# ShahzaibAhmad05/NextSearch-api

Hardware: AMD Instinct MI355X
Metric: queries/sec at k=10 over 1M-doc index; achieved HBM GB/s vs peak (higher is better)
Workload: dtype f32

## Files before the change

### include/nextsearch_hip.h

```cpp
#ifndef NEXTSEARCH_HIP_H
#define NEXTSEARCH_HIP_H

#include <stdint.h>

#ifdef __cplusplus
extern "C" {
#endif

#define NS_OK            0
#define NS_E_INVAL      -1
#define NS_E_NODEVICE   -2
#define NS_E_HIP        -3
#define NS_E_NOMEM      -4
#define NS_E_STATE      -5

#define NS_MAX_K        100u

#define NS_FLAG_OR      0u
#define NS_FLAG_AND     1u
#define NS_INFO_IMPACTS 0x100u
#define NS_INFO_PACKED  0x200u
#define NS_INFO_SHARED  0x800u
#define NS_INFO_PRUNED  0x400u

typedef struct ns_ctx   ns_ctx;
typedef struct ns_seg   ns_seg;
typedef struct ns_batch ns_batch;

typedef struct ns_term_ref {
    uint32_t seg_id;
    uint32_t count;
    uint64_t byte_off;
    float    idf;
    float    qweight;
} ns_term_ref;

typedef struct ns_query_desc {
    uint32_t term_begin;
    uint32_t term_count;
} ns_query_desc;

typedef struct ns_hit {
    float    score;
    uint32_t seg_id;
    uint32_t doc_id;
} ns_hit;

typedef struct ns_batch_info {
    uint64_t postings;
    uint64_t algo_bytes;
    uint32_t n_queries;
    uint32_t n_items;
    uint32_t n_term_refs;
    uint32_t tile_docs;
    uint32_t k;
    uint32_t flags;
    float    last_score_kernel_ms;
    float    last_total_ms;
    uint32_t timed_runs;
    uint32_t shared_lists;
    double   sum_score_kernel_ms;
    double   sum_total_ms;
    uint64_t shared_postings;
} ns_batch_info;

int  ns_ctx_create(int device, ns_ctx** out);
void ns_ctx_destroy(ns_ctx* ctx);
int  ns_ctx_set_stream(ns_ctx* ctx, void* hip_stream);
const char* ns_last_error(ns_ctx* ctx);
const char* ns_device_name(ns_ctx* ctx);

int ns_segment_upload(ns_ctx* ctx, uint32_t seg_id, uint32_t n_docs, float avgdl,
                      const uint32_t* doc_len, const void* postings, uint64_t nbytes, ns_seg** out);
int ns_segment_release(ns_ctx* ctx, ns_seg* seg);
int ns_segment_upload_begin(ns_ctx* ctx, uint32_t seg_id, uint32_t n_docs, float avgdl, const uint32_t* doc_len,
                            uint64_t total_nbytes, ns_seg** out);
int ns_segment_upload_append(ns_ctx* ctx, ns_seg* seg, const void* bytes, uint64_t nbytes);
int ns_segment_upload_end(ns_ctx* ctx, ns_seg* seg);

int ns_segment_build_impacts(ns_ctx* ctx, ns_seg* seg, const uint64_t* byte_off, const uint32_t* counts,
                             const float* idfs, uint32_t n_lists);
int ns_ctx_set_overlap(ns_ctx* ctx, int on);
int ns_ctx_set_host_threads(ns_ctx* ctx, uint32_t n);
int ns_segment_build_packed(ns_ctx* ctx, ns_seg* seg);
int ns_ctx_use_packed(ns_ctx* ctx, int mode);
int ns_ctx_use_impacts(ns_ctx* ctx, int on);
int ns_segment_build_skips(ns_ctx* ctx, ns_seg* seg, const uint64_t* byte_off, const uint32_t* counts, uint32_t n_lists);
int ns_segment_filter(ns_ctx* ctx, ns_seg* src, uint32_t new_seg_id, const uint32_t* keep_bits, const uint64_t* byte_off,
                      const uint32_t* counts, uint32_t n_lists, uint64_t* new_byte_off_out, uint32_t* new_counts_out,
                      void* postings_out, uint64_t* kept_postings_out, float* device_ms_out, ns_seg** out);
int ns_ctx_use_skips(ns_ctx* ctx, int on);
int ns_segment_build_blockmax(ns_ctx* ctx, ns_seg* seg, const uint64_t* byte_off, const uint32_t* counts,
                              const float* idfs, uint32_t n_lists);
int ns_ctx_use_pruning(ns_ctx* ctx, int on);
int ns_ctx_use_merge(ns_ctx* ctx, int on);
int ns_ctx_share_scores(ns_ctx* ctx, int mode);

int ns_ctx_share_rows(ns_ctx* ctx, int mode);
int ns_batch_row_stats(ns_batch* b, uint32_t out[4]);

int ns_search_batch(ns_ctx* ctx, const ns_query_desc* queries, const ns_term_ref* terms,
                    uint32_t n_queries, uint32_t k, ns_hit* hits_out, uint32_t* nhits_out,
                    uint64_t* found_out, uint32_t flags);

int  ns_batch_prepare(ns_ctx* ctx, const ns_query_desc* queries, const ns_term_ref* terms,
                      uint32_t n_queries, uint32_t k, uint32_t flags, ns_batch** out);
int  ns_batch_bind_outputs(ns_batch* b, void* d_hits, void* d_nhits, void* d_found);
#define NS_RUN_TIMED 1
#define NS_RUN_FETCH 2
int  ns_batch_run(ns_batch* b, int run_flags);
void* ns_batch_stream(ns_batch* b);
int  ns_batch_gap_ms(ns_batch* prev, ns_batch* next, float* ms);
int  ns_batch_sync(ns_batch* b);
int  ns_batch_fetch(ns_batch* b, ns_hit* hits_out, uint32_t* nhits_out, uint64_t* found_out);
int  ns_batch_get_info(ns_batch* b, ns_batch_info* info);
void ns_batch_destroy(ns_batch* b);

typedef struct ns_sem ns_sem;
int ns_sem_upload(ns_ctx* ctx, const float* vecs, uint32_t n_rows, uint32_t dim, ns_sem** out);
int ns_sem_release(ns_ctx* ctx, ns_sem* sem);
int ns_sem_topk(ns_ctx* ctx, ns_sem* sem, const float* qvecs, uint32_t n_q, uint32_t topk, float min_sim,
                const uint32_t* ban_off, const uint32_t* ban_rows, uint32_t* rows_out, float* sims_out,
                uint32_t* counts_out, float* device_ms_out);

typedef struct ns_ac ns_ac;
int ns_ac_upload(ns_ctx* ctx, const uint8_t* pool, const uint64_t* offsets, const uint32_t* scores, uint32_t n_terms, ns_ac** out);
int ns_ac_suggest(ns_ctx* ctx, ns_ac* ac, const uint8_t* prefix_bytes, const uint32_t* prefix_offsets, uint32_t n_q, uint32_t L,
                  uint32_t* idx_out, uint32_t* count_out, float* device_ms_out);
int ns_ac_release(ns_ctx* ctx, ns_ac* ac);

#define NS_FUZZY_MAX_LEN   64u
#define NS_FUZZY_MAX_EDITS 2u
int ns_ac_build_fuzzy(ns_ctx* ctx, ns_ac* ac, float* device_ms_out);
int ns_ac_fuzzy(ns_ctx* ctx, ns_ac* ac, const uint8_t* term_bytes, const uint32_t* term_offsets, uint32_t n_q,
                const uint8_t* max_edits, uint32_t prefix_len, uint32_t L, uint32_t* idx_out, uint8_t* dist_out,
                uint32_t* count_out, float* device_ms_out);

int ns_ac_fuzzy_prefix(ns_ctx* ctx, ns_ac* ac, const uint8_t* prefix_bytes, const uint32_t* prefix_offsets, uint32_t n_q,
                       const uint8_t* max_edits, uint32_t prefix_len, uint32_t L, uint32_t* idx_out, uint8_t* dist_out,
                       uint32_t* count_out, float* device_ms_out);

int ns_merge_rank_rows(ns_ctx* ctx, const void* d_hits, const void* d_nhits, const void* d_found, uint32_t n_ranks,
                       uint32_t n_queries, uint32_t k, const uint32_t* d_seg_map, uint32_t seg_map_stride,
                       void* d_out_hits, void* d_out_nhits, void* d_out_found);

int ns_invert_forward(ns_ctx* ctx, const uint32_t* doc_term_counts, uint32_t n_docs, const uint32_t* pairs,
                      uint64_t n_pairs, uint32_t n_terms, uint32_t* df_out, void* postings_out, uint64_t* kept_out,
                      float* device_ms_out);
int ns_segment_upload_inverted(ns_ctx* ctx, ns_seg* seg, const uint32_t* doc_term_counts, const uint32_t* pairs,
                               uint64_t n_pairs, uint32_t n_terms, uint32_t* df_out, void* postings_out,
                               uint64_t* kept_out, float* device_ms_out);

#define NS_E_ARG NS_E_INVAL
typedef struct ns_forward ns_forward;
typedef struct ns_forward_info {
    uint32_t struct_size;
    uint32_t kept_docs;
    uint32_t n_terms;
    uint32_t n_docs;
    uint64_t n_pairs;
    uint64_t term_bytes;
    uint64_t n_tokens;
    uint64_t kept_tokens;
    uint64_t device_bytes;
    float    device_ms;
    uint32_t pad;
} ns_forward_info;
int ns_forward_build(ns_ctx* ctx, const uint8_t* text, uint64_t text_bytes, const uint64_t* offsets, uint32_t n_docs,
                     ns_forward** out);
int ns_forward_get_info(const ns_forward* fwd, ns_forward_info* info);
int ns_forward_fetch(ns_forward* fwd, uint32_t* kept_docs_out, uint32_t* doc_len_out, uint32_t* counts_out,
                     uint32_t* pairs_out, uint8_t* term_bytes_out, uint64_t* term_offsets_out);
void ns_forward_destroy(ns_forward* fwd);

typedef struct ns_forward_src {
    uint32_t n_docs;  const uint32_t* doc_len;  const uint32_t* counts;
    uint64_t n_pairs; const uint32_t* pairs;
    uint32_t n_terms; const uint8_t* term_bytes; const uint64_t* term_offsets;
} ns_forward_src;
int ns_forward_merge(ns_ctx* ctx, const ns_forward_src* src, uint32_t n_src, ns_forward** out);
int ns_forward_invert(ns_forward* fwd, uint32_t* df_out, void* postings_out, uint64_t* kept_out, float* device_ms_out);
uint32_t ns_compact_doc_cut(void);
// ... 73 lines not shown
```

### nextsearch-api_amd/csrc/ns_api.hip

```cpp
#include <hip/hip_runtime.h>

#include <algorithm>
#include <cmath>
#include <cstdarg>
#include <cstdio>
#include <cstdlib>
#include <cstring>
#include <string>
#include <vector>

#include "../../include/nextsearch_hip.h"
#include "ns_internal.h"
#include "ns_plan.hpp"
#include "ns_kernels.hip"
#include "ns_wave_kernel.hip"
#include "ns_driver_kernel.hip"
#include "ns_prune_kernel.hip"
#include "ns_merge_kernel.hip"
#include "ns_tile_kernel.hip"
#include "ns_row_kernel.hip"
#include "ns_invert.hip"
#include "ns_ingest.hip"
#include "ns_compact.hip"
#include "ns_delete.hip"
#include "ns_filter.hip"
#include "ns_facet.hip"
#include "ns_similar.hip"
#include "ns_sorted.hip"
#include "ns_boolean.hip"
#include "ns_boolean_sets.hip"
#include "ns_sem.hip"
#include "ns_suggest.hip"
#include "ns_fuzzy.hip"

using namespace ns;

static_assert(sizeof(ns_hit) == sizeof(Hit), "ns_hit layout");


struct ns_seg {
    ns_ctx* ctx = nullptr;
    uint32_t id = 0;
    uint32_t n_docs = 0;
    uint64_t n_postings = 0;
    uint2* d_postings = nullptr;
    float* d_norm = nullptr;
    float* d_pnorm = nullptr;
    bool norm_safe = false;
    float avgdl = 0.0f;
    bool pending = false;
    uint64_t filled = 0;
    uint32_t* d_len = nullptr;
    void* pin[2] = {nullptr, nullptr};
    hipEvent_t ev[2] = {nullptr, nullptr};
    int stage_k = 0;
    uint32_t* d_packed = nullptr;
    uint2* d_pk_hdr = nullptr;
    float* d_pk_scores = nullptr;
    uint16_t* d_nidx = nullptr;
    float* d_ntab = nullptr;
    uint32_t n_norms = 0;
    uint2* d_impacts = nullptr;
    uint32_t* d_skips = nullptr;
    std::vector<uint32_t*> skip_retired;
    uint64_t skip_cap = 0, skip_used = 0;
    uint32_t skip_entries() const { return (n_docs + kSkipDocs - 1) / kSkipDocs + 2; }
    float* d_blockmax = nullptr;
    std::vector<float*> bmx_retired;
    uint64_t bmx_cap = 0, bmx_used = 0;
    SegLists lists;
};

struct ns_ctx {
    struct Block { void* p; size_t n; };
    std::vector<Block> pool;
    size_t pool_bytes = 0;
    int device = 0;
    hipStream_t own_stream = nullptr;
    hipStream_t stream = nullptr;
    hipStream_t alt_stream = nullptr;
    hipStream_t pull_stream = nullptr;
    bool overlap = false, flip = false;
    hipStream_t row_stream = nullptr;
    std::string err;
    std::string devname;
    std::vector<ns_seg*> segs;
    std::vector<ns_seg*> pending_uploads;
    void* h_up = nullptr;
    size_t h_up_cap = 0;
    hipEvent_t up_done = nullptr;
    bool up_busy = false;
    void* h_down = nullptr;
    size_t h_down_cap = 0;
    struct ns_batch* down_owner = nullptr;
    struct DownSlot { void* p = nullptr; size_t cap = 0; bool busy = false; };
    std::vector<DownSlot> down_slots;
    PlanSettings cfg;
    ShareRegistry share;
    BatchPlan plan;
    std::vector<ns_ac*> acs;
    std::vector<ns_forward*> fwds;
    bool cp_inplace = true;
    std::vector<ns_docterms*> dts;
};

static thread_local std::string g_create_err;
static void ac_free_fwd(ns_ac* ac);
static void forward_orphan_fwd(ns_forward* f);
static void docterms_orphan_fwd(ns_docterms* h);
static void seg_free_device_fwd(ns_seg* s);
static void seg_free_staging_fwd(ns_seg* s);

static int fail(ns_ctx* ctx, int code, const char* fmt, ...) {
    va_list ap;
    va_start(ap, fmt);
    (ctx ? ctx->err : g_create_err) = vformat(fmt, ap);
    va_end(ap);
    return code;
}

#define HIPCHK(ctx, call)                                                                         \
    do {                                                                                          \
        hipError_t e_ = (call);                                                                   \
        if (e_ != hipSuccess)                                                                     \
            return fail((ctx), NS_E_HIP, "%s failed: %s (%s:%d)", #call, hipGetErrorString(e_), __FILE__, __LINE__); \
    } while (0)

template <int CB, int TMAX, bool IMP, int PK>
static void launch_uscore(bool and_mode, uint32_t n_items, hipStream_t st, const DevWItem* items, const DevTerm* terms,
                          const DevSeg* segs, Hit* hits, uint32_t* nhits, uint64_t* found, uint32_t K) {
    dim3 grid((n_items + kUscoreWavesPerBlock - 1) / kUscoreWavesPerBlock), block(64 * kUscoreWavesPerBlock);
    if (and_mode)
        hipLaunchKernelGGL((k_uscore<512, 192, true, CB, TMAX, IMP, PK>), grid, block, 0, st, items, n_items, terms, segs, hits, nhits, found, K);
    else
        hipLaunchKernelGGL((k_uscore<512, 192, false, CB, TMAX, IMP, PK>), grid, block, 0, st, items, n_items, terms, segs, hits, nhits, found, K);
}
template <int CB, int TMAX>
static void launch_uscore(bool and_mode, bool imp, int pk, uint32_t n_items, hipStream_t st, const DevWItem* items,
                          const DevTerm* terms, const DevSeg* segs, Hit* hits, uint32_t* nhits, uint64_t* found, uint32_t K) {
    if (imp && pk) launch_uscore<CB, TMAX, true, 1>(and_mode, n_items, st, items, terms, segs, hits, nhits, found, K);
    else if (imp) launch_uscore<CB, TMAX, true, 0>(and_mode, n_items, st, items, terms, segs, hits, nhits, found, K);
    else if (pk == 2) launch_uscore<CB, TMAX, false, 2>(and_mode, n_items, st, items, terms, segs, hits, nhits, found, K);
    else if (pk == 1) launch_uscore<CB, TMAX, false, 1>(and_mode, n_items, st, items, terms, segs, hits, nhits, found, K);
    else launch_uscore<CB, TMAX, false, 0>(and_mode, n_items, st, items, terms, segs, hits, nhits, found, K);
}

template <int HK, int FB>
static void launch_dscore(bool and_mode, uint32_t n_items, hipStream_t st, const DevWItem* items, const DevTerm* terms,
                          const DevSeg* segs, Hit* hits, uint32_t* nhits, uint64_t* found, uint32_t K) {
    dim3 grid((n_items + 3) / 4), block(256);
    if (and_mode)
        hipLaunchKernelGGL((k_dscore<HK, FB, true>), grid, block, 0, st, items, n_items, terms, segs, hits, nhits, found, K);
    else
        hipLaunchKernelGGL((k_dscore<HK, FB, false>), grid, block, 0, st, items, n_items, terms, segs, hits, nhits, found, K);
}

template <int TD>
static void launch_tscore(bool and_mode, uint32_t n_items, hipStream_t st, const DevWItem* items, const DevTerm* terms,
                          const DevSeg* segs, Hit* hits, uint32_t* nhits, uint64_t* found, uint32_t K) {
    dim3 grid((n_items + 3) / 4), block(256);
    if (and_mode)
        hipLaunchKernelGGL((k_tscore<TD, true>), grid, block, 0, st, items, n_items, terms, segs, hits, nhits, found, K);
    else
        hipLaunchKernelGGL((k_tscore<TD, false>), grid, block, 0, st, items, n_items, terms, segs, hits, nhits, found, K);
}

template <int NT, int SPT, int U>
static void launch_score(bool and_mode, uint32_t n_items, hipStream_t st, const DevItem* items, const DevTerm* terms,
                         const DevSeg* segs, const uint32_t* bounds, Hit* hits, uint32_t* nhits, uint64_t* found,
                         uint32_t K) {
    if (and_mode)
        hipLaunchKernelGGL((k_score<NT, SPT, U, true>), dim3(n_items), dim3(NT), 0, st, items, terms, segs, bounds, hits, nhits, found, K);
    else
        hipLaunchKernelGGL((k_score<NT, SPT, U, false>), dim3(n_items), dim3(NT), 0, st, items, terms, segs, bounds, hits, nhits, found, K);
}

extern "C" int ns_ctx_create(int device, ns_ctx** out) {
    if (!out) return fail(nullptr, NS_E_INVAL, "ns_ctx_create: out is NULL");
    *out = nullptr;
    int ndev = 0;
    hipError_t e = hipGetDeviceCount(&ndev);
    if (e != hipSuccess || ndev <= 0)
        return fail(nullptr, NS_E_NODEVICE, "no HIP device available (%s); this library has no CPU fallback",
                    e == hipSuccess ? "device count 0" : hipGetErrorString(e));
    if (device < 0 || device >= ndev) return fail(nullptr, NS_E_INVAL, "device %d out of range [0,%d)", device, ndev);
    e = hipSetDevice(device);
    if (e != hipSuccess) return fail(nullptr, NS_E_NODEVICE, "hipSetDevice(%d): %s", device, hipGetErrorString(e));
    hipDeviceProp_t prop;
    e = hipGetDeviceProperties(&prop, device);
    if (e != hipSuccess) return fail(nullptr, NS_E_NODEVICE, "hipGetDeviceProperties: %s", hipGetErrorString(e));
    ns_ctx* ctx = new ns_ctx();
    ctx->device = device;
    ctx->devname = std::string(prop.gcnArchName) + " " + prop.name;
    ctx->cfg.n_cus = prop.multiProcessorCount;
    e = hipStreamCreateWithFlags(&ctx->own_stream, hipStreamNonBlocking);
    if (e != hipSuccess) {
        int rc = fail(nullptr, NS_E_HIP, "hipStreamCreate: %s", hipGetErrorString(e));
        delete ctx;
        return rc;
    }
    ctx->stream = ctx->own_stream;
    if (const char* om = std::getenv("NS_ORDER_MODE")) ctx->cfg.order_mode = std::atoi(om);
    if (const char* kp = std::getenv("NS_KEY_PCT")) {
        unsigned a = 100, b = 100, c = 100, d = 100;
        if (std::sscanf(kp, "%u,%u,%u,%u", &a, &b, &c, &d) >= 1) { ctx->cfg.key_pct[0] = a; ctx->cfg.key_pct[1] = b; ctx->cfg.key_pct[2] = c; ctx->cfg.key_pct[3] = d; }
    }
    if (const char* td = std::getenv("NS_TILE_DENS64")) ctx->cfg.tile_dens64 = (uint32_t)std::max(1, std::atoi(td));
    if (const char* um = std::getenv("NS_MERGE")) ctx->cfg.use_merge = std::atoi(um) != 0;
    if (const char* mr = std::getenv("NS_MERGE_RATIO")) ctx->cfg.merge_ratio = (uint32_t)std::max(1, std::atoi(mr));
    if (const char* sm = std::getenv("NS_SHARE")) ctx->cfg.share_mode = std::max(0, std::min(2, std::atoi(sm)));
    if (const char* sr = std::getenv("NS_SHARE_RATIO")) ctx->cfg.share_ratio = (uint32_t)std::max(1, std::atoi(sr));
    if (const char* sp = std::getenv("NS_SHARE_MIN")) ctx->cfg.share_min_postings = (uint64_t)std::max(0ll, std::atoll(sp));
    ctx->cfg.row_mode = 1;
    if (const char* rm = std::getenv("NS_SHARE_ROWS")) ctx->cfg.row_mode = std::max(0, std::min(2, std::atoi(rm)));
    if (const char* ru = std::getenv("NS_ROW_MIN_USERS")) ctx->cfg.row_min_users = (uint32_t)std::max(1, std::atoi(ru));
    if (const char* rc = std::getenv("NS_ROW_CELL")) ctx->cfg.row_cell_postings = (uint32_t)std::max(1, std::atoi(rc));
    {
        const char* rf = std::getenv("NS_ROW_FORK");
        if ((!rf || std::atoi(rf) != 0) && hipStreamCreateWithFlags(&ctx->row_stream, hipStreamNonBlocking) != hipSuccess) { ctx->row_stream = nullptr; (void)hipGetLastError(); }
    }
    if (const char* oc = std::getenv("NS_ORDER_COARSE")) { ctx->cfg.order_coarse = std::max(0, std::min(11, std::atoi(oc))); ctx->cfg.order_coarse_forced = true; }
    if (hipStreamCreateWithFlags(&ctx->alt_stream, hipStreamNonBlocking) != hipSuccess) { ctx->alt_stream = nullptr; (void)hipGetLastError(); }
    {
        int lo_pri = 0, hi_pri = 0;
        (void)hipDeviceGetStreamPriorityRange(&lo_pri, &hi_pri);
        if (hipStreamCreateWithPriority(&ctx->pull_stream, hipStreamNonBlocking, hi_pri) != hipSuccess) { ctx->pull_stream = nullptr; (void)hipGetLastError(); }
    }
    *out = ctx;
    return NS_OK;
}

extern "C" void ns_ctx_destroy(ns_ctx* ctx) {
    if (!ctx) return;
    (void)hipSetDevice(ctx->device);
    (void)hipStreamSynchronize(ctx->stream);
    if (ctx->alt_stream) (void)hipStreamSynchronize(ctx->alt_stream);
    if (ctx->pull_stream) (void)hipStreamSynchronize(ctx->pull_stream);
    if (ctx->row_stream) (void)hipStreamSynchronize(ctx->row_stream);
    for (ns_seg* s : ctx->segs) {
        if (!s) continue;
        seg_free_device_fwd(s);
        delete s;
    }
    for (ns_seg* s : ctx->pending_uploads) {
        seg_free_staging_fwd(s);
        seg_free_device_fwd(s);
        delete s;
    }
    for (ns_ac* ac : ctx->acs) ac_free_fwd(ac);
    for (ns_forward* f : ctx->fwds) forward_orphan_fwd(f);
    for (ns_docterms* h : ctx->dts) docterms_orphan_fwd(h);
    for (auto& blk : ctx->pool) (void)hipFree(blk.p);
    if (ctx->h_up) (void)hipHostFree(ctx->h_up);
    if (ctx->h_down) (void)hipHostFree(ctx->h_down);
    for (auto& ds : ctx->down_slots) if (ds.p) (void)hipHostFree(ds.p);
    if (ctx->up_done) (void)hipEventDestroy(ctx->up_done);
    if (ctx->own_stream) (void)hipStreamDestroy(ctx->own_stream);
    if (ctx->alt_stream) (void)hipStreamDestroy(ctx->alt_stream);
    if (ctx->pull_stream) (void)hipStreamDestroy(ctx->pull_stream);
    if (ctx->row_stream) (void)hipStreamDestroy(ctx->row_stream);
    delete ctx;
}

extern "C" int ns_ctx_set_stream(ns_ctx* ctx, void* hip_stream) {
    if (!ctx) return fail(nullptr, NS_E_INVAL, "ns_ctx_set_stream: ctx is NULL");
    ctx->stream = hip_stream ? (hipStream_t)hip_stream : ctx->own_stream;
    return NS_OK;
}

extern "C" const char* ns_last_error(ns_ctx* ctx) { return ctx ? ctx->err.c_str() : g_create_err.c_str(); }
extern "C" const char* ns_device_name(ns_ctx* ctx) { return ctx ? ctx->devname.c_str() : ""; }

extern "C" int ns_set_tuning(ns_ctx* ctx, uint32_t variant, uint32_t min_items, uint32_t split_postings) {
    if (!ctx) return fail(nullptr, NS_E_INVAL, "ns_set_tuning: ctx is NULL");
    if (variant >= kNumVariants || kVariants[variant].nt == 0) return fail(ctx, NS_E_INVAL, "unknown kernel variant %u", variant);
#ifndef NS_VARIANTS
    if (variant != 0) return fail(ctx, NS_E_INVAL, "kernel variant %u exists only in the variants build (make -C nextsearch-api_amd variants)", variant);
#endif
    ctx->cfg.variant = variant;
    ctx->cfg.min_items = min_items;
    ctx->cfg.split_postings = split_postings;
    return NS_OK;
}

static constexpr size_t kPadPostings = 256;
static constexpr size_t kStageChunk = 32u << 20;

static void seg_free_staging(ns_seg* s) {
    for (int i = 0; i < 2; i++) {
        if (s->pin[i]) (void)hipHostFree(s->pin[i]);
        if (s->ev[i]) (void)hipEventDestroy(s->ev[i]);
        s->pin[i] = nullptr; s->ev[i] = nullptr;
    }
    if (s->d_len) (void)hipFree(s->d_len);
    s->d_len = nullptr;
}
static void seg_free_device(ns_seg* s);
static void seg_free_device_fwd(ns_seg* s) { seg_free_device(s); }
static void seg_free_staging_fwd(ns_seg* s) { seg_free_staging(s); }
static void seg_free_device(ns_seg* s) {
    (void)hipFree(s->d_postings);
    (void)hipFree(s->d_norm);
    (void)hipFree(s->d_pnorm);
    (void)hipFree(s->d_impacts);
    (void)hipFree(s->d_packed);
    (void)hipFree(s->d_pk_hdr);
    (void)hipFree(s->d_pk_scores);
    (void)hipFree(s->d_nidx);
    (void)hipFree(s->d_ntab);
    (void)hipFree(s->d_skips);
    for (uint32_t* p : s->skip_retired) (void)hipFree(p);
    s->skip_retired.clear();
    (void)hipFree(s->d_blockmax);
    for (float* p : s->bmx_retired) (void)hipFree(p);
    s->bmx_retired.clear();
    s->d_blockmax = nullptr; s->bmx_cap = s->bmx_used = 0; s->lists.bmx.clear();
    s->d_skips = nullptr; s->skip_cap = s->skip_used = 0; s->lists.skip.clear();
    s->d_postings = nullptr; s->d_norm = nullptr; s->d_pnorm = nullptr; s->d_impacts = nullptr; s->d_packed = nullptr;
    s->d_pk_hdr = nullptr; s->d_pk_scores = nullptr; s->d_nidx = nullptr; s->d_ntab = nullptr;
}
static hipError_t seg_stage(ns_ctx* ctx, ns_seg* s, void* dst, const void* src, size_t n) {
    size_t off = 0;
    while (off < n) {
        const size_t c = std::min(kStageChunk, n - off);
        const int k = s->stage_k;
        hipError_t r = hipEventSynchronize(s->ev[k]);
        if (r != hipSuccess) return r;
        std::memcpy(s->pin[k], (const char*)src + off, c);
        r = hipMemcpyAsync((char*)dst + off, s->pin[k], c, hipMemcpyHostToDevice, ctx->stream);
        if (r != hipSuccess) return r;
        r = hipEventRecord(s->ev[k], ctx->stream);
        if (r != hipSuccess) return r;
        off += c;
        s->stage_k ^= 1;
    }
    return hipSuccess;
}

extern "C" int ns_segment_upload_begin(ns_ctx* ctx, uint32_t seg_id, uint32_t n_docs, float avgdl, const uint32_t* doc_len,
                                       uint64_t nbytes, ns_seg** out) {
    if (!ctx) return fail(nullptr, NS_E_INVAL, "ns_segment_upload: ctx is NULL");
    if (!out) return fail(ctx, NS_E_INVAL, "ns_segment_upload_begin: out is NULL");
    *out = nullptr;
    if (seg_id >= (1u << 20)) return fail(ctx, NS_E_INVAL, "seg_id %u too large", seg_id);
    if (nbytes % 8 != 0) return fail(ctx, NS_E_INVAL, "posting payload of %llu bytes is not a whole number of {u32,u32} pairs", (unsigned long long)nbytes);
    if (nbytes / 8 >= (1ull << 32)) return fail(ctx, NS_E_INVAL, "segment has %llu postings; this build indexes postings with 32 bits (split the segment)", (unsigned long long)(nbytes / 8));
    if (n_docs && !doc_len) return fail(ctx, NS_E_INVAL, "null doc_len/postings");
    if (seg_id < ctx->segs.size() && ctx->segs[seg_id]) return fail(ctx, NS_E_INVAL, "segment %u already uploaded", seg_id);
    HIPCHK(ctx, hipSetDevice(ctx->device));

    ns_seg* s = new ns_seg();
    s->ctx = ctx;
    s->id = seg_id;
    s->n_docs = n_docs;
    s->n_postings = nbytes / 8;
    s->avgdl = avgdl;
    s->pending = true;
    auto cleanup = [&]() { seg_free_staging(s); seg_free_device(s); delete s; };

    hipError_t e;
    if ((e = hipMalloc((void**)&s->d_postings, nbytes + kPadPostings * 8)) != hipSuccess) { cleanup(); return fail(ctx, NS_E_NOMEM, "hipMalloc postings (%llu B): %s", (unsigned long long)nbytes, hipGetErrorString(e)); }
    if ((e = hipMalloc((void**)&s->d_norm, (size_t)std::max<uint32_t>(n_docs, 1) * 4)) != hipSuccess) { cleanup(); return fail(ctx, NS_E_NOMEM, "hipMalloc norm: %s", hipGetErrorString(e)); }
    if ((e = hipMalloc((void**)&s->d_pnorm, nbytes / 2 + kPadPostings * 4)) != hipSuccess) { cleanup(); return fail(ctx, NS_E_NOMEM, "hipMalloc per-posting norms (%llu B): %s", (unsigned long long)(nbytes / 2), hipGetErrorString(e)); }
    if ((e = hipMalloc((void**)&s->d_len, (size_t)std::max<uint32_t>(n_docs, 1) * 4)) != hipSuccess) { cleanup(); return fail(ctx, NS_E_NOMEM, "hipMalloc doc_len: %s", hipGetErrorString(e)); }
    for (int i = 0; i < 2; i++)
        if (hipHostMalloc(&s->pin[i], kStageChunk, hipHostMallocDefault) != hipSuccess || hipEventCreateWithFlags(&s->ev[i], hipEventDisableTiming) != hipSuccess) {
            cleanup();
            return fail(ctx, NS_E_NOMEM, "pinned staging allocation failed");
        }
    e = hipMemsetAsync((char*)s->d_postings + nbytes, 0xFF, kPadPostings * 8, ctx->stream);
    if (e == hipSuccess) e = hipMemsetAsync((char*)s->d_pnorm + nbytes / 2, 0, kPadPostings * 4, ctx->stream);
    if (e == hipSuccess && n_docs) e = seg_stage(ctx, s, s->d_len, doc_len, (size_t)n_docs * 4);
    if (e == hipSuccess && n_docs) {
        hipLaunchKernelGGL(k_norm, dim3((n_docs + 255) / 256), dim3(256), 0, ctx->stream, s->d_len, s->d_norm, n_docs, avgdl);
        e = hipGetLastError();
    }
    if (e == hipSuccess && n_docs) {
        uint32_t max_len = 0;
        for (uint32_t i = 0; i < n_docs; i++) max_len = std::max(max_len, doc_len[i]);
        std::vector<uint32_t> uniq;
        std::vector<uint16_t> nidx;
        if (max_len < (1u << 24)) {
            std::vector<uint32_t> rank((size_t)max_len + 1, 0u);
            for (uint32_t i = 0; i < n_docs; i++) rank[doc_len[i]] = 1u;
            for (uint32_t v = 0; v <= max_len; v++)
                if (rank[v]) { rank[v] = (uint32_t)uniq.size(); uniq.push_back(v); }
            if (uniq.size() <= 65536) {
                nidx.resize(n_docs);
                for (uint32_t i = 0; i < n_docs; i++) nidx[i] = (uint16_t)rank[doc_len[i]];
            }
        } else {
            uniq.assign(doc_len, doc_len + n_docs);
            std::sort(uniq.begin(), uniq.end());
            uniq.erase(std::unique(uniq.begin(), uniq.end()), uniq.end());
            if (uniq.size() <= 65536) {
                nidx.resize(n_docs);
                for (uint32_t i = 0; i < n_docs; i++) nidx[i] = (uint16_t)(std::lower_bound(uniq.begin(), uniq.end(), doc_len[i]) - uniq.begin());
            }
        }
        if (!nidx.empty()) {
// ... 222 lines not shown
    }
}

extern "C" int ns_ctx_share_scores(ns_ctx* ctx, int mode) {
    if (!ctx) return fail(nullptr, NS_E_INVAL, "ns_ctx_share_scores: ctx is NULL");
    if (mode < 0 || mode > 2) return fail(ctx, NS_E_INVAL, "ns_ctx_share_scores: mode %d outside [0, 2]", mode);
    ctx->cfg.share_mode = mode;
    return NS_OK;
}

extern "C" int ns_ctx_share_rows(ns_ctx* ctx, int mode) {
    if (!ctx) return fail(nullptr, NS_E_INVAL, "ns_ctx_share_rows: ctx is NULL");
    if (mode < 0 || mode > 2) return fail(ctx, NS_E_INVAL, "ns_ctx_share_rows: mode %d outside [0, 2]", mode);
    ctx->cfg.row_mode = mode;
    return NS_OK;
}

extern "C" int ns_segment_build_packed(ns_ctx* ctx, ns_seg* seg) {
    if (!ctx || !seg) return fail(ctx, NS_E_INVAL, "ns_segment_build_packed: null argument");
    if (seg->pending || seg->id >= ctx->segs.size() || ctx->segs[seg->id] != seg) return fail(ctx, NS_E_INVAL, "segment does not belong to this ctx");
    if (seg->d_packed || !seg->n_postings) return NS_OK;
    if (!seg->d_nidx) return fail(ctx, NS_E_INVAL, "ns_segment_build_packed: segment %u has more than 65536 distinct document lengths; its norms do not fit a 16-bit index", seg->id);
    HIPCHK(ctx, hipSetDevice(ctx->device));
    const uint64_t n_blocks = (seg->n_postings + kPkBlock - 1) / kPkBlock;
    hipError_t e = hipMalloc((void**)&seg->d_packed, (n_blocks + 2) * kPkStrideDwords * 4);
    if (e == hipSuccess) e = hipMalloc((void**)&seg->d_pk_hdr, (n_blocks + 2) * sizeof(uint2));
    if (e == hipSuccess) e = hipMemsetAsync(seg->d_packed + n_blocks * kPkStrideDwords, 0, 2 * kPkStrideDwords * 4, ctx->stream);
    if (e == hipSuccess) e = hipMemsetAsync(seg->d_pk_hdr + n_blocks, 0, 2 * sizeof(uint2), ctx->stream);
    if (e == hipSuccess) {
        hipLaunchKernelGGL(k_pack, dim3((uint32_t)n_blocks), dim3(64), 0, ctx->stream, seg->d_postings, seg->d_nidx, seg->d_packed, seg->d_pk_hdr,
                           seg->n_postings, seg->n_docs, (uint32_t)n_blocks);
        e = hipGetLastError();
    }
    if (e == hipSuccess) e = hipStreamSynchronize(ctx->stream);
    if (e == hipSuccess) e = seg_fill_pk_scores(ctx, seg);
    if (e != hipSuccess) {
        (void)hipFree(seg->d_packed); (void)hipFree(seg->d_pk_hdr);
        seg->d_packed = nullptr; seg->d_pk_hdr = nullptr;
        return fail(ctx, e == hipErrorOutOfMemory ? NS_E_NOMEM : NS_E_HIP, "ns_segment_build_packed: %s", hipGetErrorString(e));
    }
    return NS_OK;
}

__global__ void __launch_bounds__(256) k_skip_fill(uint32_t* __restrict__ sk, const uint32_t* __restrict__ starts, const uint32_t* __restrict__ counts,
                                                   uint32_t per_list) {
    const uint32_t l = blockIdx.y;
    const uint32_t endp = starts[l] + counts[l];
    for (uint32_t i = blockIdx.x * 256 + threadIdx.x; i < per_list; i += gridDim.x * 256) sk[(uint64_t)l * per_list + i] = endp;
}
__global__ void __launch_bounds__(256) k_skip_build(const uint2* __restrict__ postings, uint32_t* __restrict__ sk, const uint32_t* __restrict__ starts,
                                                    const uint32_t* __restrict__ counts, uint32_t per_list) {
    const uint32_t l = blockIdx.y;
    const uint32_t first = starts[l], n = counts[l];
    uint32_t* row = sk + (uint64_t)l * per_list;
    const uint32_t cells = per_list - 2;
    for (uint32_t i = blockIdx.x * 256 + threadIdx.x; i < n; i += gridDim.x * 256) {
        const uint32_t d = postings[first + i].x / kSkipDocs;
        uint32_t c0 = 0;
        if (i) {
            const uint32_t dp = postings[first + i - 1].x / kSkipDocs;
            c0 = dp + 1;
        }
        for (uint32_t c = c0; c <= d && c <= cells; c++) row[c] = first + i;
    }
}
__global__ void __launch_bounds__(256) k_skip_check(const uint2* __restrict__ postings, const uint32_t* __restrict__ sk, const uint32_t* __restrict__ starts,
                                                    const uint32_t* __restrict__ counts, uint32_t per_list, uint32_t* __restrict__ bad) {
    const uint32_t l = blockIdx.y;
    const uint32_t first = starts[l], endp = first + counts[l];
    const uint32_t* row = sk + (uint64_t)l * per_list;
    bool b = false;
    for (uint32_t i = blockIdx.x * 256 + threadIdx.x; i + 1 < per_list; i += gridDim.x * 256) {
        const uint32_t a = row[i], z = row[i + 1];
        if (a > z || a < first || z > endp) b = true;
        if (i == 0 && a != first) b = true;
        if (i + 2 == per_list && (z != endp || a != endp)) b = true;
        if (i + 2 < per_list && a < z) {
            if (postings[a].x / kSkipDocs != i || postings[z - 1].x / kSkipDocs != i) b = true;
        }
    }
    if (b) bad[l] = 1u;
}

extern "C" int ns_segment_build_skips(ns_ctx* ctx, ns_seg* seg, const uint64_t* byte_off, const uint32_t* counts, uint32_t n_lists) {
    if (!ctx || !seg) return fail(ctx, NS_E_INVAL, "ns_segment_build_skips: null argument");
    if (seg->pending || seg->id >= ctx->segs.size() || ctx->segs[seg->id] != seg) return fail(ctx, NS_E_INVAL, "segment does not belong to this ctx");
    if (n_lists && (!byte_off || !counts)) return fail(ctx, NS_E_INVAL, "null list arrays");
    if (!n_lists || !seg->n_postings || !seg->n_docs) return NS_OK;
    HIPCHK(ctx, hipSetDevice(ctx->device));
    if (int rc = check_lists(ctx, seg, byte_off, counts, n_lists)) return rc;
    struct L { uint32_t first, count; };
    std::vector<L> lists;
    lists.reserve(n_lists);
    for (uint32_t i = 0; i < n_lists; i++)
        if (counts[i] && !seg->lists.skip_of((uint32_t)(byte_off[i] / 8), counts[i])) lists.push_back({(uint32_t)(byte_off[i] / 8), counts[i]});
    std::sort(lists.begin(), lists.end(), [](const L& a, const L& b) { return a.first < b.first || (a.first == b.first && a.count < b.count); });
    lists.erase(std::unique(lists.begin(), lists.end(), [](const L& a, const L& b) { return a.first == b.first; }), lists.end());
    if (lists.empty()) return NS_OK;
    const uint32_t per_list = seg->skip_entries();
    const size_t n = lists.size();
    const uint64_t need = seg->skip_used + (uint64_t)n * per_list;
    if (need >= (1ull << 32) - 1) return fail(ctx, NS_E_INVAL, "ns_segment_build_skips: %llu table entries do not fit 32 bits", (unsigned long long)need);
    hipError_t e = hipSuccess;
    if (need > seg->skip_cap) {
        uint32_t* bigger = nullptr;
        const uint64_t cap = std::max<uint64_t>(need, seg->skip_cap * 2);
        e = hipMalloc((void**)&bigger, cap * 4);
        if (e != hipSuccess) return fail(ctx, NS_E_NOMEM, "hipMalloc skip tables (%llu B): %s", (unsigned long long)(cap * 4), hipGetErrorString(e));
        if (seg->d_skips) {
            e = hipMemcpyAsync(bigger, seg->d_skips, seg->skip_used * 4, hipMemcpyDeviceToDevice, ctx->stream);
            seg->skip_retired.push_back(seg->d_skips);
        }
        seg->d_skips = bigger;
        seg->skip_cap = cap;
        if (e != hipSuccess) return fail(ctx, NS_E_HIP, "ns_segment_build_skips: %s", hipGetErrorString(e));
    }
    std::vector<uint32_t> h(n * 3, 0u);
    for (size_t i = 0; i < n; i++) { h[i] = lists[i].first; h[n + i] = lists[i].count; }
    uint32_t* d_tmp = nullptr;
    e = hipMalloc((void**)&d_tmp, n * 12);
    if (e == hipSuccess) e = hipMemcpyAsync(d_tmp, h.data(), n * 12, hipMemcpyHostToDevice, ctx->stream);
    uint32_t* base = seg->d_skips + seg->skip_used;
    if (e == hipSuccess) {
        const dim3 g1((per_list + 255) / 256 > 64 ? 64 : (per_list + 255) / 256, (uint32_t)n);
        hipLaunchKernelGGL(k_skip_fill, g1, dim3(256), 0, ctx->stream, base, d_tmp, d_tmp + n, per_list);
        uint32_t cmax = 0;
        for (const auto& l : lists) cmax = std::max(cmax, l.count);
        const dim3 g2(std::min<uint32_t>((cmax + 255) / 256, 1024u), (uint32_t)n);
        hipLaunchKernelGGL(k_skip_build, g2, dim3(256), 0, ctx->stream, seg->d_postings, base, d_tmp, d_tmp + n, per_list);
        hipLaunchKernelGGL(k_skip_check, g1, dim3(256), 0, ctx->stream, seg->d_postings, base, d_tmp, d_tmp + n, per_list, d_tmp + 2 * n);
        e = hipGetLastError();
    }
    std::vector<uint32_t> bad(n, 1u);
    if (e == hipSuccess) e = hipMemcpyAsync(bad.data(), d_tmp + 2 * n, n * 4, hipMemcpyDeviceToHost, ctx->stream);
    if (e == hipSuccess) e = hipStreamSynchronize(ctx->stream);
    (void)hipFree(d_tmp);
    if (e != hipSuccess) return fail(ctx, NS_E_HIP, "ns_segment_build_skips: %s", hipGetErrorString(e));
    for (size_t i = 0; i < n; i++)
        if (!bad[i] && !seg->lists.skip.find(lists[i].first)) seg->lists.skip.put(lists[i].first, {lists[i].count, (uint32_t)(seg->skip_used + i * per_list)});
    seg->skip_used = need;
    return NS_OK;
}

extern "C" int ns_segment_build_blockmax(ns_ctx* ctx, ns_seg* seg, const uint64_t* byte_off, const uint32_t* counts, const float* idfs, uint32_t n_lists) {
    if (!ctx || !seg) return fail(ctx, NS_E_INVAL, "ns_segment_build_blockmax: null argument");
    if (seg->pending || seg->id >= ctx->segs.size() || ctx->segs[seg->id] != seg) return fail(ctx, NS_E_INVAL, "segment does not belong to this ctx");
    if (n_lists && (!byte_off || !counts || !idfs)) return fail(ctx, NS_E_INVAL, "null list arrays");
    if (!n_lists || !seg->n_postings) return NS_OK;
    HIPCHK(ctx, hipSetDevice(ctx->device));
    if (int rc = check_lists(ctx, seg, byte_off, counts, n_lists)) return rc;
    struct L { uint32_t first, count; float idf; uint32_t entry; };
    std::vector<L> lists;
    lists.reserve(n_lists);
    for (uint32_t i = 0; i < n_lists; i++) {
        uint32_t ib; std::memcpy(&ib, &idfs[i], 4);
        if (counts[i] && !seg->lists.bmx_of((uint32_t)(byte_off[i] / 8), counts[i], ib)) lists.push_back({(uint32_t)(byte_off[i] / 8), counts[i], idfs[i], 0u});
    }
    std::sort(lists.begin(), lists.end(), [](const L& a, const L& b) { return a.first < b.first; });
    lists.erase(std::unique(lists.begin(), lists.end(), [](const L& a, const L& b) { return a.first == b.first; }), lists.end());
    if (lists.empty()) return NS_OK;
    uint64_t need = seg->bmx_used;
    uint32_t bmax_blocks = 0;
    for (auto& l : lists) {
        const uint32_t nb = (l.count + kBmxBlock - 1) / kBmxBlock;
        l.entry = (uint32_t)need;
        need += nb;
        bmax_blocks = std::max(bmax_blocks, nb);
    }
    if (need + 64 >= (1ull << 32) - 1) return fail(ctx, NS_E_INVAL, "ns_segment_build_blockmax: %llu entries do not fit 32 bits", (unsigned long long)need);
    hipError_t e = hipSuccess;
    if (need + 64 > seg->bmx_cap) {
        float* bigger = nullptr;
        const uint64_t cap = std::max<uint64_t>(need + 64, seg->bmx_cap * 2);
        e = hipMalloc((void**)&bigger, cap * 4);
        if (e != hipSuccess) return fail(ctx, NS_E_NOMEM, "hipMalloc block maxima (%llu B): %s", (unsigned long long)(cap * 4), hipGetErrorString(e));
        e = hipMemsetAsync(bigger, 0, cap * 4, ctx->stream);
        if (e == hipSuccess && seg->d_blockmax) {
            e = hipMemcpyAsync(bigger, seg->d_blockmax, seg->bmx_used * 4, hipMemcpyDeviceToDevice, ctx->stream);
            seg->bmx_retired.push_back(seg->d_blockmax);
        }
        seg->d_blockmax = bigger;
        seg->bmx_cap = cap;
        if (e != hipSuccess) return fail(ctx, NS_E_HIP, "ns_segment_build_blockmax: %s", hipGetErrorString(e));
    }
    const size_t n = lists.size();
    std::vector<uint32_t> h(n * 4);
    for (size_t i = 0; i < n; i++) {
        h[i] = lists[i].first; h[n + i] = lists[i].count;
        std::memcpy(&h[2 * n + i], &lists[i].idf, 4);
        h[3 * n + i] = lists[i].entry;
    }
    uint32_t* d_tmp = nullptr;
    e = hipMalloc((void**)&d_tmp, n * 16);
    if (e == hipSuccess) e = hipMemcpyAsync(d_tmp, h.data(), n * 16, hipMemcpyHostToDevice, ctx->stream);
    if (e == hipSuccess) {
        for (size_t l0 = 0; l0 < n; l0 += 32768) {
            const uint32_t ny = (uint32_t)std::min<size_t>(32768, n - l0);
            hipLaunchKernelGGL(k_blockmax, dim3(std::min<uint32_t>(std::max<uint32_t>(bmax_blocks, 1u), 256u), ny), dim3(64), 0, ctx->stream,
                               seg->d_postings, seg->d_pnorm, seg->d_blockmax, d_tmp + l0, d_tmp + n + l0, (const float*)(d_tmp + 2 * n + l0), d_tmp + 3 * n + l0);
        }
        e = hipGetLastError();
    }
    if (e == hipSuccess) e = hipStreamSynchronize(ctx->stream);
    (void)hipFree(d_tmp);
    if (e != hipSuccess) return fail(ctx, NS_E_HIP, "ns_segment_build_blockmax: %s", hipGetErrorString(e));
    seg->bmx_used = need;
    for (const auto& l : lists) {
        uint32_t ib; std::memcpy(&ib, &l.idf, 4);
        seg->lists.bmx.put(l.first, {l.count, ib, l.entry});
    }
    return NS_OK;
}

extern "C" int ns_ctx_use_merge(ns_ctx* ctx, int on) {
    if (!ctx) return NS_E_INVAL;
    ctx->cfg.use_merge = on != 0;
    return NS_OK;
}

extern "C" int ns_ctx_use_pruning(ns_ctx* ctx, int on) {
    if (!ctx) return NS_E_INVAL;
    ctx->cfg.use_pruning = on != 0;
    return NS_OK;
// ... 542 lines not shown
    if (!b) return NS_E_INVAL;
    ns_ctx* ctx = b->ctx;
    HIPCHK(ctx, hipSetDevice(ctx->device));
    HIPCHK(ctx, hipStreamSynchronize(b->st));
    return batch_collect_timings(b);
}

extern "C" int ns_batch_fetch(ns_batch* b, ns_hit* hits_out, uint32_t* nhits_out, uint64_t* found_out) {
    if (!b) return NS_E_INVAL;
    ns_ctx* ctx = b->ctx;
    if (!b->ran) return fail(ctx, NS_E_STATE, "ns_batch_fetch before ns_batch_run");
    HIPCHK(ctx, hipSetDevice(ctx->device));
    hipStream_t st = b->st;
    const bool own_outputs = b->o_hits == b->d_hits && b->o_nhits == b->d_nhits && b->o_found == b->d_found;
    if (b->fetch_enqueued && b->done_recorded && own_outputs) {
        HIPCHK(ctx, hipEventSynchronize(b->done));
        int rc = batch_collect_timings(b);
        if (rc != NS_OK) return rc;
        if (b->Q) {
            const char* h = (ctx->down_owner == b) ? (const char*)ctx->h_down : (const char*)ctx->down_slots[(size_t)b->down_slot].p;
            if (hits_out) std::memcpy(hits_out, h, (size_t)b->Q * b->K * sizeof(Hit));
            if (nhits_out) std::memcpy(nhits_out, h + b->off_nhits, (size_t)b->Q * 4);
            if (found_out) std::memcpy(found_out, h + b->off_found, (size_t)b->Q * 8);
        }
        if (b->down_slot >= 0) { ctx->down_slots[(size_t)b->down_slot].busy = false; b->down_slot = -1; }
        b->fetch_enqueued = false;
        return NS_OK;
    }
    if (b->Q && own_outputs && ctx->down_owner == b) {
        int rc = ns_batch_sync(b);
        if (rc != NS_OK) return rc;
        const char* h = (const char*)ctx->h_down;
        if (hits_out) std::memcpy(hits_out, h, (size_t)b->Q * b->K * sizeof(Hit));
        if (nhits_out) std::memcpy(nhits_out, h + b->off_nhits, (size_t)b->Q * 4);
        if (found_out) std::memcpy(found_out, h + b->off_found, (size_t)b->Q * 8);
        return NS_OK;
    }
    if (b->Q && own_outputs && !ctx->down_owner && b->out_span <= kStageMaxBytes) {
        if (ctx->h_down_cap < b->out_span) {
            if (ctx->h_down) (void)hipHostFree(ctx->h_down);
            ctx->h_down = nullptr; ctx->h_down_cap = 0;
            const size_t cap = std::max<size_t>(b->out_span + b->out_span / 2, 1 << 16);
            if (hipHostMalloc(&ctx->h_down, cap, hipHostMallocDefault) == hipSuccess) ctx->h_down_cap = cap;
            else { ctx->h_down = nullptr; (void)hipGetLastError(); }
        }
        if (ctx->h_down_cap >= b->out_span) {
            HIPCHK(ctx, hipMemcpyAsync(ctx->h_down, b->d_hits, b->out_span, hipMemcpyDeviceToHost, st));
            int rc = ns_batch_sync(b);
            if (rc != NS_OK) return rc;
            const char* h = (const char*)ctx->h_down;
            if (hits_out) std::memcpy(hits_out, h, (size_t)b->Q * b->K * sizeof(Hit));
            if (nhits_out) std::memcpy(nhits_out, h + b->off_nhits, (size_t)b->Q * 4);
            if (found_out) std::memcpy(found_out, h + b->off_found, (size_t)b->Q * 8);
            return NS_OK;
        }
    }
    if (b->Q) {
        if (hits_out) HIPCHK(ctx, hipMemcpyAsync(hits_out, b->o_hits, (size_t)b->Q * b->K * sizeof(Hit), hipMemcpyDeviceToHost, st));
        if (nhits_out) HIPCHK(ctx, hipMemcpyAsync(nhits_out, b->o_nhits, (size_t)b->Q * 4, hipMemcpyDeviceToHost, st));
        if (found_out) HIPCHK(ctx, hipMemcpyAsync(found_out, b->o_found, (size_t)b->Q * 8, hipMemcpyDeviceToHost, st));
    }
    return ns_batch_sync(b);
}

extern "C" int ns_batch_get_info(ns_batch* b, ns_batch_info* info) {
    if (!b || !info) return NS_E_INVAL;
    info->postings = b->postings;
    info->algo_bytes = b->postings * 8;
    info->n_queries = b->Q;
    info->n_items = b->n_items + b->n_witems + b->n_ritems + b->n_pitems;
    info->n_term_refs = b->n_terms;
    info->tile_docs = b->tile_docs;
    info->k = b->K;
    info->flags = b->flags | (b->imp ? NS_INFO_IMPACTS : 0u) | (b->pk ? NS_INFO_PACKED : 0u) | (b->pruned ? NS_INFO_PRUNED : 0u) |
                  (b->shared ? NS_INFO_SHARED : 0u);
    info->shared_lists = b->n_share;
    info->shared_postings = b->share_postings;
    info->last_score_kernel_ms = b->last_score_ms;
    info->last_total_ms = b->last_total_ms;
    info->timed_runs = b->timed_runs;
    info->sum_score_kernel_ms = b->sum_score_ms;
    info->sum_total_ms = b->sum_total_ms;
    return NS_OK;
}

extern "C" int ns_batch_row_stats(ns_batch* b, uint32_t out[4]) {
    if (!b || !out) return NS_E_INVAL;
    ns_ctx* ctx = b->ctx;
    const bool rows = b->n_pitems && b->n_ritems && b->variant == 0;
    out[0] = rows ? b->n_pitems : 0u; out[1] = rows ? b->n_ritems : 0u; out[2] = 0u; out[3] = 0u;
    if (rows && b->ran) {
        HIPCHK(ctx, hipSetDevice(ctx->device));
        HIPCHK(ctx, hipMemcpyAsync(out + 2, b->d_row_stats, 8, hipMemcpyDeviceToHost, b->st));
        HIPCHK(ctx, hipStreamSynchronize(b->st));
    }
    return NS_OK;
}

extern "C" int ns_search_batch(ns_ctx* ctx, const ns_query_desc* queries, const ns_term_ref* terms, uint32_t n_queries,
                               uint32_t k, ns_hit* hits_out, uint32_t* nhits_out, uint64_t* found_out, uint32_t flags) {
    ns_batch* b = nullptr;
    int rc = ns_batch_prepare(ctx, queries, terms, n_queries, k, flags, &b);
    if (rc != NS_OK) return rc;
    rc = ns_batch_run(b, 0);
    if (rc == NS_OK) rc = ns_batch_fetch(b, hits_out, nhits_out, found_out);
    ns_batch_destroy(b);
    return rc;
}


static int invert_run(ns_ctx* ctx, const uint32_t* doc_term_counts, uint32_t n_docs, const uint32_t* pairs,
                      uint64_t n_pairs, uint32_t n_terms, uint32_t* df_out, void* postings_out, uint64_t* kept_out,
                      float* device_ms_out, ns_seg* adopt, const uint2* dev_pairs = nullptr) {
    if (!ctx) return fail(nullptr, NS_E_INVAL, "ns_invert_forward: ctx is NULL");
    if ((n_docs && !doc_term_counts) || (n_pairs && !pairs && !dev_pairs) || (n_terms && !df_out) || !kept_out) return fail(ctx, NS_E_INVAL, "ns_invert_forward: null argument");
    if (n_pairs >= (1ull << 32) - kIvTile) return fail(ctx, NS_E_INVAL, "ns_invert_forward: %llu pairs; this build indexes pairs with 32 bits (split the segment)", (unsigned long long)n_pairs);
    if (n_terms == 0xFFFFFFFFu) return fail(ctx, NS_E_INVAL, "ns_invert_forward: n_terms too large");
    *kept_out = 0;
    if (device_ms_out) *device_ms_out = 0.0f;
    std::vector<uint64_t> prefix((size_t)n_docs + 1, 0);
    for (uint32_t d = 0; d < n_docs; d++) prefix[d + 1] = prefix[d] + doc_term_counts[d];
    if (prefix[n_docs] != n_pairs) return fail(ctx, NS_E_INVAL, "ns_invert_forward: the per-document counts sum to %llu, not to n_pairs = %llu", (unsigned long long)prefix[n_docs], (unsigned long long)n_pairs);
    if (n_terms) std::memset(df_out, 0, (size_t)n_terms * 4);
    if (!n_pairs) return NS_OK;
    if (!postings_out && !adopt) return fail(ctx, NS_E_INVAL, "ns_invert_forward: postings_out is NULL");
    HIPCHK(ctx, hipSetDevice(ctx->device));
    hipStream_t st = ctx->stream;
    const uint32_t n = (uint32_t)n_pairs;
    const uint32_t n_tiles = (n + kIvTile - 1) / kIvTile;
    int bits = 1;
    while (bits < 32 && n_terms > 1 && ((n_terms - 1) >> bits) != 0) bits++;
    const int passes = std::max(1, (bits + 10) / 11);
    int pbits[3] = {8, 8, 8};
    {
        int left = bits;
        for (int p = 0; p < passes; p++) {
            const int share = (left + (passes - p) - 1) / (passes - p);
            pbits[p] = std::min(11, std::max(8, share));
            left = std::max(0, left - pbits[p]);
        }
    }
    size_t m_max = 0;
    for (int p = 0; p < passes; p++) m_max = std::max(m_max, ((size_t)1 << pbits[p]) * n_tiles);
    const uint32_t scan_blocks_max = (uint32_t)((m_max + 1023) / 1024);

    uint2 *d_pairs = nullptr, *d_vals[2] = {nullptr, nullptr};
    uint32_t *d_keys[2] = {nullptr, nullptr}, *d_df = nullptr, *d_first = nullptr, *d_hist = nullptr, *d_sums = nullptr, *d_kept = nullptr;
    uint64_t* d_prefix = nullptr;
    uint2* d_tile_docs = nullptr;
    std::vector<uint32_t> tile_docs((size_t)n_tiles * 2);
    {
        uint32_t d = 0;
        auto doc_of = [&](uint64_t i) { while (d + 1 < n_docs && prefix[d + 1] <= i) d++; return d; };
        for (uint32_t t = 0; t < n_tiles; t++) {
            const uint64_t i0 = (uint64_t)t * kIvTile, i1 = std::min<uint64_t>(i0 + kIvTile, n) - 1;
            tile_docs[2 * (size_t)t] = doc_of(i0);
            tile_docs[2 * (size_t)t + 1] = doc_of(i1);
        }
    }
    hipEvent_t ev0 = nullptr, ev1 = nullptr;
    hipError_t e = hipSuccess;
    auto chk = [&](hipError_t r) { if (e == hipSuccess) e = r; };
    size_t off = 0;
    auto place = [&](size_t bytes) { const size_t o = off; off = (off + std::max<size_t>(bytes, 1) + 255) & ~(size_t)255; return o; };
    const size_t nt1 = (size_t)std::max<uint32_t>(n_terms, 1);
    const size_t o_pairs = place(dev_pairs ? 1 : (size_t)n * 8), o_v0 = place((size_t)n * 8), o_v1 = place(passes > 1 ? (size_t)n * 8 : 1);
// ... 2402 lines not shown
```

### nextsearch-api_amd/csrc/ns_driver_kernel.hip

```cpp
#pragma once
#include <hip/hip_runtime.h>
#include <stdint.h>

#include "ns_internal.h"
#include "ns_wave_kernel.hip"

namespace ns {

#ifdef NS_COUNT
constexpr int kNsCnt = 32;
__device__ unsigned long long g_ns_cnt[kNsCnt];
#define NS_CNT(i, v) cnt_[(i)] += (unsigned long long)(v)
#else
#define NS_CNT(i, v)
#endif

template <bool IMP, int PKM>
__device__ __forceinline__ void pk_decode_round(const DevSeg& seg, const uint32_t blk, const int lane, uint32_t (&doc)[4], float (&tf)[4],
                                                float (&nr)[4], uint32_t (&sbits)[4]) {
    const gp_u32 pb = (gp_u32)seg.packed + (size_t)blk * kPkStrideDwords + (uint32_t)lane;
    const uint32_t d0 = pb[kPkDoc], d1 = pb[kPkDoc + 64];
    uint32_t t = 0, na = 0, nb = 0;
    if (IMP) {
        const gp_f32 sc = (gp_f32)seg.pk_scores + (size_t)blk * kPkBlock + (uint32_t)lane;
#pragma unroll
        for (int c = 0; c < 4; c++) { sbits[c] = __float_as_uint(sc[c * 64]); tf[c] = 0.0f; nr[c] = 0.0f; }
    } else {
        t = pb[kPkTf];
        if (PKM == 2) { na = pb[kPkNormA]; nb = pb[kPkNormB]; }
        else {
            const gp_f32 np = (gp_f32)seg.pnorm + (size_t)blk * kPkBlock + (uint32_t)lane;
#pragma unroll
            for (int c = 0; c < 4; c++) nr[c] = np[c * 64];
        }
    }
    typedef const __attribute__((address_space(4))) uint32_t* cp_u32;
    const cp_u32 hp = (cp_u32)(const void*)(seg.pk_hdr + blk);
    const uint32_t base = hp[0];
    const uint32_t code = hp[1];
    if (code == 0u) {
#pragma unroll
        for (int c = 0; c < 4; c++) doc[c] = base + ((d0 >> (8 * c)) & 255u);
    } else if (code == 1u) {
        doc[0] = base + (d0 & 0xFFFFu); doc[1] = base + (d0 >> 16);
        doc[2] = base + (d1 & 0xFFFFu); doc[3] = base + (d1 >> 16);
    } else {
        doc[0] = d0; doc[1] = d1;
        doc[2] = pb[kPkDoc + 128]; doc[3] = pb[kPkDoc + 192];
    }
    if (!IMP) {
        uint32_t tfi[4];
#pragma unroll
        for (int c = 0; c < 4; c++) tfi[c] = (t >> (8 * c)) & 255u;
        const uint32_t nt_ = ~t;
        if (wballot(((nt_ - 0x01010101u) & t & 0x80808080u) != 0u) != 0ull) {
            const gp_u2 raw = (gp_u2)seg.postings + (size_t)blk * kPkBlock + (uint32_t)lane;
#pragma unroll
            for (int c = 0; c < 4; c++)
                if (tfi[c] == 255u) { const nat_u2 pv = raw[c * 64]; tfi[c] = pv.y; }
        }
        if (PKM == 2) {
            const gp_f32 ntab = (gp_f32)seg.ntab;
            nr[0] = ntab[na & 0xFFFFu]; nr[1] = ntab[na >> 16];
            nr[2] = ntab[nb & 0xFFFFu]; nr[3] = ntab[nb >> 16];
        }
#pragma unroll
        for (int c = 0; c < 4; c++) { tf[c] = (float)tfi[c]; sbits[c] = 0u; }
    }
}

__device__ __forceinline__ uint64_t lane_span(uint32_t lo, uint32_t hi) {
    const uint64_t upto_hi = hi >= 64u ? ~0ull : ((1ull << hi) - 1ull);
    const uint64_t upto_lo = lo >= 64u ? ~0ull : ((1ull << lo) - 1ull);
    return upto_hi & ~upto_lo;
}

struct RowArgs { const Hit* hits; uint32_t nhits; uint32_t dterm; uint32_t* stats; };

template <int NB, int FB, bool AND, int CB = 256, bool IMP = false, int PK = 0, bool ROW = false>
__device__ __forceinline__ bool dscore_body(const DevWItem& it, const DevTerm* __restrict__ terms, const DevSeg* __restrict__ segs,
                                            uint32_t* ent, float* vals, uint8_t* mcnt, uint64_t* cand, uint4* tab, uint32_t* aux,
                                            Hit* __restrict__ out_hits, uint32_t* __restrict__ out_nhits,
                                            uint64_t* __restrict__ out_found, uint32_t K, const int lane, const RowArgs ra = RowArgs{}) {
    static_assert(!ROW || (FB == 64 && !AND && IMP && PK == 0), "the row consumer is the thin OR body over shared term scores");
    constexpr int FE = FB / 64;
    constexpr int DE = 4;
    constexpr uint32_t EMPTY = 0u;
    constexpr int LOG2NB = (NB == 64) ? 6 : (NB == 128 ? 7 : 8);
    constexpr uint32_t MAXSPAN = (1u << (LOG2NB + 15)) - 1u;
#define NS_BUCKET(doc) ((uint32_t)__builtin_amdgcn_ubfe(__umul24((doc) - lo, bm), 16u, (uint32_t)LOG2NB))
#define NS_TAG(doc) (0x8000u | (((doc) - lo) & 0x7FFFu))
#define NS_IDENT(doc, bkt) ((NS_TAG(doc) << 16) | ((bkt) << 8))
    static_assert(NB == 64 || NB == 128 || NB == 256, "NB must be 64, 128 or 256");
    static_assert(FB % 64 == 0 && FB >= 64 && FB <= 256 && FB <= 2 * NB, "FB must be a multiple of 64, at most 256 and 2*NB");
    uint4* ent4 = reinterpret_cast<uint4*>(ent);

#ifdef NS_COUNT
    const unsigned long long cyc_t0_ = __builtin_readcyclecounter();
#endif
    const DevSeg seg = segs[it.seg];
    const uint32_t T = it.term_count;
    const bool fast_div = (__builtin_amdgcn_readfirstlane((int)it.whole) & 8) != 0;
    const bool signed_in = (__builtin_amdgcn_readfirstlane((int)it.whole) & 16) != 0;
    const gp_u2 postings = (gp_u2)seg.postings;
    const gp_f32 pnorm = (gp_f32)seg.pnorm;
    const gp_u2 stream = IMP ? (gp_u2)seg.impacts : postings;

    {
        const uint4 empty4 = make_uint4(EMPTY, EMPTY, EMPTY, EMPTY);
#pragma unroll
        for (int g = 0; g < NB / 64; g++) ent4[g * 64 + lane] = empty4;
#pragma unroll
        for (int g = 0; g < FB / 64; g++) {
            vals[g * 64 + lane] = 0.0f;
            if (AND) mcnt[g * 64 + lane] = 0;
        }
    }

    uint32_t base = 0, cur = 0, end = 0, idf_bits = 0, wq_bits = 0;
    if ((uint32_t)lane < T) {
        const DevTerm tm = terms[it.term_begin + lane];
        base = (uint32_t)tm.list_off;
        idf_bits = __float_as_uint(tm.idf);
        wq_bits = __float_as_uint(tm.weight);
        const uint2 r = item_list_range(it, seg, tm);
        cur = r.x + base;
        end = r.y + base;
        tab[lane] = make_uint4(idf_bits, wq_bits, 0u, 0u);
    }
    uint32_t dl;
    {
        const uint32_t remv = end - cur;
        const uint32_t mx = wave_max_dpp(remv);
        dl = (uint32_t)__builtin_ctzll(wballot(remv == mx && (uint32_t)lane < T) | (1ull << 63));
        if (dl >= T) dl = 0;
    }
    if constexpr (ROW) dl = ra.dterm;
    uint32_t d_cur = rdlane(cur, dl);
    const uint32_t d_end = rdlane(end, dl);
    const float d_idf = __uint_as_float(rdlane(idf_bits, dl));
    const float d_wq = __uint_as_float(rdlane(wq_bits, dl));
    uint32_t Rf = 0;
    {
        const uint32_t r32 = ((uint32_t)lane == dl) ? 0u : (end - cur);
        for (uint32_t t = 0; t < T; t++) {
            const uint32_t v = rdlane(r32, t);
            Rf = (Rf + v < Rf) ? 0xFFFFFFFFu : (Rf + v);
        }
    }
    if ((uint32_t)lane == dl) { cur = end; }

#ifdef NS_COUNT
    unsigned long long cnt_[kNsCnt] = {};
    cnt_[16] = __builtin_readcyclecounter() - cyc_t0_; cnt_[17] = 0;
    NS_CNT(0, 1);
    NS_CNT(10, T);
#endif
    uint32_t lo = it.doc_lo;
    const uint32_t last_doc = it.doc_hi - 1;
    WaveTopK<CB> top(cand, K, lane);
    uint32_t found_s = 0;
    float r_sc = 0.0f;
    uint32_t r_doc = 0xFFFFFFFFu, row_hits = 0;
    uint64_t r_left = 0ull;
    bool row_complete = false;
    gp_u32 d_skips = nullptr;
    if constexpr (ROW) {
        const uint32_t nrow = min(ra.nhits, kRowLen);
        const Hit rh = ra.hits[lane];
        r_sc = rh.score; r_doc = rh.doc;
        r_left = lane_span(0u, nrow);
        found_s = d_end - d_cur;
        row_complete = nrow == d_end - d_cur;
        d_skips = (gp_u32)seg.skips + (terms[it.term_begin + dl].skip - 1u);
        NS_CNT(19, 1);
    }

    constexpr uint32_t WSLACK = (FB == 64) ? kWinSlackThin : kWinSlackGen;
    uint32_t w_n = 0, e_n = 0xFFFFFFFFu;
#define NS_PLAN_FOREIGN()                                                                          \
    {                                                                                              \
        const uint32_t rem_ = end - cur;               \
        const uint32_t nact_ = (uint32_t)__popcll(wballot(rem_ > 0));                             \
        const uint32_t c_ = foreign_slack(WSLACK, (uint32_t)FB, nact_, Rf);            \
        const float scale_ = foreign_scale(c_, (uint32_t)FB, nact_, __builtin_amdgcn_rcpf((float)max(Rf, 1u))); \
        const uint32_t w_ = foreign_window(rem_, c_, scale_);                                      \
        const bool probe_ = w_ < rem_;                                                             \
        const uint32_t pi_ = probe_ ? (cur + w_ - 1u) : 0u;                                        \
        const nat_u2 pv_ = postings[pi_];      \
        w_n = (rem_ > 0) ? w_ : 0u;                                                                \
        e_n = probe_ ? pv_.x : 0xFFFFFFFFu;                                                        \
    }
    NS_PLAN_FOREIGN();
    wave_sync();
    for (;;) {
        top.begin_step();
        NS_CNT(1, 1);
        const uint32_t w = w_n;
        const uint32_t e = e_n;
        const uint32_t incl = wave_incl_scan_dpp(w);
        const uint32_t total = rdlane(incl, 63);
        uint32_t hi = wave_min_dpp(e);
        const uint32_t span_hi = (last_doc - lo > MAXSPAN) ? (lo + MAXSPAN) : last_doc;
        const bool span_clamped = hi > span_hi && span_hi != last_doc;
        hi = min(hi, span_hi);
        NS_CNT(27, span_clamped ? 1 : 0);
        uint32_t bm;
        {
            const uint32_t spn1 = (hi >= lo ? hi - lo : 0u) + 1u;
            bm = (uint32_t)((float)((uint32_t)NB << 16) * __builtin_amdgcn_rcpf((float)spn1));
            bm = (uint32_t)__builtin_amdgcn_readfirstlane((int)bm);
            while ((uint64_t)bm * spn1 > (uint64_t)((uint32_t)NB << 16)) bm--;
            while ((uint64_t)(bm + 1u) * spn1 <= (uint64_t)((uint32_t)NB << 16)) bm++;
            bm = min(bm, 0xFFFFFFu);
        }

        uint32_t ftj[FE];
        float fx[FE];
        bool fok[FE], fmine[FE];
        uint32_t fdoc[FE];
        uint32_t tb_min = 0, tb_max = 0;
#pragma unroll
        for (int j = 0; j < FE; j++) { ftj[j] = 0; fx[j] = 0.0f; fok[j] = false; fmine[j] = false; fdoc[j] = 0; }
        if (total > 0) {
            if ((uint32_t)lane < T) reinterpret_cast<uint2*>(tab + lane)[1] = make_uint2(cur - (incl - w), cur);
            if (T > 8 && (uint32_t)lane < T) aux[lane] = incl;
            wave_sync();
            NS_CNT(26, T > 8 ? 1 : 0);
            if (T <= 8) {
                for (uint32_t t = 0; t + 1 < T; t++) {
                    const uint32_t sp = rdlane(incl, t);
#pragma unroll
                    for (int j = 0; j < FE; j++) ftj[j] += ((uint32_t)(j * 64 + lane) >= sp) ? 1u : 0u;
                }
            } else {
#pragma unroll
                for (int j = 0; j < FE; j++) {
                    const uint32_t p = min((uint32_t)(j * 64 + lane), total - 1u);
                    uint32_t a = 0, b = T - 1;
                    while (a < b) {
                        const uint32_t m = (a + b) >> 1;
                        if (aux[m] > p) b = m; else a = m + 1;
                    }
                    ftj[j] = a;
                }
                wave_sync();
            }
            nat_u2 pst[FE];
            float nrm[FE];
            uint32_t pidx[FE];
#pragma unroll
            for (int j = 0; j < FE; j++) {
                const uint32_t p = (uint32_t)(j * 64 + lane);
                const bool inb = p < total;
                ftj[j] = inb ? ftj[j] : 0u;
                pidx[j] = tab[ftj[j]].z + (inb ? p : 0u);
                pst[j] = stream[pidx[j]];
// ... 119 lines not shown
                }
                wave_sync();
            }
#pragma unroll
            for (int j = 0; j < FE; j++) {
                if ((uint32_t)(j * 64) >= total) continue;
                bool pending = fok[j] && !fmine[j];
                if (wballot(pending) == 0ull) continue;
                const uint32_t me = (uint32_t)(j * 64 + lane);
                uint32_t b = NS_BUCKET(fdoc[j]);
                const uint32_t mine = NS_IDENT(fdoc[j], b) | me;
                const bool todo = pending;
                uint32_t slot = 0, own = 0;
                bool scan = pending;
                uint32_t pos = 0;
                for (int round = 0; round < 8 * NB; round++) {
                    if (wballot(pending) == 0ull) break;
                    NS_CNT(6, 1);
                    if (wballot(scan) != 0ull) {
#ifdef NS_COUNT
                        bool owner_found_ = false;
#endif
                        if (scan) {
                            const uint4 q = ent4[b];
                            const uint32_t tmin = min(min(q.x ^ mine, q.y ^ mine), min(q.z ^ mine, q.w ^ mine));
                            pos = (q.x >> 31) + (q.y >> 31) + (q.z >> 31) + (q.w >> 31);
                            if (tmin < 256u) { own = tmin ^ me; pending = false; }
#ifdef NS_COUNT
                            owner_found_ = tmin < 256u;
#endif
                            scan = false;
                        }
                        NS_CNT(24, (uint32_t)__popcll(wballot(owner_found_)));
                    }
                    const bool try_store = pending && pos < 4;
                    if (try_store) ent[b * 4 + pos] = mine;
                    wave_sync();
                    if (try_store) {
                        const uint32_t back = ent[b * 4 + pos];
                        if ((back ^ mine) < 256u) { slot = b * 4 + pos; own = back & 255u; pending = false; }
                        else pos++;
                    } else if (pending) {
                        b = (b + 1) & (uint32_t)(NB - 1);
                        scan = true;
                    }
                    NS_CNT(22, (uint32_t)__popcll(wballot(pending && scan)));
                    NS_CNT(23, (uint32_t)__popcll(wballot(pending && scan && b == 0u)));
                    wave_sync();
                }
                if (todo) {
                    fmine[j] = own == me;
                    ftj[j] |= (own << 6) | (slot << 14);
                }
            }
        }

#define NS_FOREIGN_RMW(ta, tb)                                                                     \
        for (uint32_t tt = (ta); tt <= (tb); tt++) {                                               \
            if (tt == dl) continue;                                                                \
            NS_CNT(7, 1);                                                                          \
            float old_[FE];                                                                        \
             \
                                    \
            _Pragma("unroll") for (int j = 0; j < FE; j++) {                                       \
                const bool c_ = fok[j] && (ftj[j] & 63u) == tt;                                    \
                old_[j] = vals[c_ ? ((ftj[j] >> 6) & 255u) : (uint32_t)(j * 64 + lane)];           \
            }                                                                                      \
            _Pragma("unroll") for (int j = 0; j < FE; j++) {                                       \
                if (fok[j] && (ftj[j] & 63u) == tt) {                                              \
                    const uint32_t o_ = (ftj[j] >> 6) & 255u;                                      \
                    vals[o_] = old_[j] + fx[j];                                                    \
                    if (AND) mcnt[o_] = (uint8_t)(mcnt[o_] + 1);                                   \
                }                                                                                  \
            }                                                                                      \
            wave_sync();                                                                           \
        }
        if (total > 0 && tb_min < dl) { NS_FOREIGN_RMW(tb_min, min(tb_max, dl - 1)); }

        if constexpr (ROW) {
            if (total > 0) {
                static_assert(FE == 1, "one foreign posting per lane");
                const bool own = fmine[0];
                const uint32_t doc = own ? fdoc[0] : lo;
                const uint32_t cell = doc / kSkipDocs;
                uint32_t a = d_skips[cell];
                uint32_t n = d_skips[cell + 1u] - a;
                bool hit = false;
                uint32_t hbits = 0u;
#pragma unroll
                for (int step = 0; step < 4; step++) {
                    const uint32_t s8 = (n + 7u) >> 3;
                    nat_u2 pv[7];
#pragma unroll
                    for (int i = 0; i < 7; i++) {
                        const uint32_t e = (uint32_t)(i + 1) * s8;
                        pv[i] = stream[a + ((e <= n && e != 0u) ? e - 1u : 0u)];
                    }
                    uint32_t c = 0u;
#pragma unroll
                    for (int i = 0; i < 7; i++) {
                        const uint32_t e = (uint32_t)(i + 1) * s8;
                        const bool valid = e <= n && e != 0u;
                        c += (valid && pv[i].x < doc) ? 1u : 0u;
                        if (valid && pv[i].x == doc) { hit = true; hbits = pv[i].y; }
                    }
                    const bool closed = c < 7u && (c + 1u) * s8 <= n;
                    a += c * s8;
                    n = (n == 0u) ? 0u : (closed ? s8 - 1u : n - c * s8);
                }
                hit = hit && own;
                if (hit) vals[lane] = vals[lane] + d_wq * __uint_as_float(hbits);
                found_s -= (uint32_t)__popcll(wballot(hit));
                NS_CNT(28, (uint32_t)__popcll(wballot(own)));
                NS_CNT(29, (uint32_t)__popcll(wballot(hit)));
                wave_sync();
            }
            const uint64_t inr = r_left & wballot(r_doc <= hi);
            if (inr != 0ull) {
                uint64_t offm = inr;
                if (total > 0) {
                    const uint32_t tag = NS_TAG(r_doc);
                    const uint32_t hb = NS_BUCKET(r_doc);
                    uint32_t b = hb;
                    uint4 q = ent4[b];
                    const uint64_t cm = wballot((q.x >> 16) == tag) | wballot((q.y >> 16) == tag) |
                                        wballot((q.z >> 16) == tag) | wballot((q.w >> 16) == tag);
                    const uint64_t go = inr & (cm | wballot(q.w != EMPTY));
                    NS_CNT(30, (uint32_t)__popcll(inr));
                    if (go != 0ull) {
                        const uint32_t ident = NS_IDENT(r_doc, hb);
                        uint32_t m = 0;
                        bool more = __builtin_amdgcn_inverse_ballot_w64(go);
                        for (int round = 0; round < NB; round++) {
                            if (wballot(more) == 0ull) break;
                            if (more) {
                                m = ((q.x ^ ident) < 256u) ? q.x : m;
                                m = ((q.y ^ ident) < 256u) ? q.y : m;
                                m = ((q.z ^ ident) < 256u) ? q.z : m;
                                m = ((q.w ^ ident) < 256u) ? q.w : m;
                                more = m == 0 && q.w != EMPTY;
                                if (more) { b = (b + 1) & (uint32_t)(NB - 1); q = ent4[b]; }
                            }
                        }
                        const uint64_t hitm = wballot(m != 0) & go;
                        offm &= ~hitm;
                        row_hits += (uint32_t)__popcll(hitm);
                        NS_CNT(31, (uint32_t)__popcll(hitm));
                    }
                }
                top.offer_mask_stream(offm, r_sc, r_doc);
                r_left &= ~inr;
            }
        }

        bool driver_progress = false;
        if constexpr (!ROW) for (;;) {
            const uint32_t remd = d_end - d_cur;
            if (remd == 0) break;
            uint32_t n;
            nat_u2 ps[DE];
            float nr[DE];
            float tfv[DE];
            uint32_t sbits[DE];
            uint32_t cnt = 0, r_hits = 0;
            NS_CNT(8, 1);
            float dx[DE];
            uint64_t dokm[DE];
            uint32_t first_pos, last_pos;
            if (PK) {
                static_assert(DE == 4, "a packed round is one block of 4 chunks");
                const uint32_t blk = d_cur >> 8;
                const uint32_t a = d_cur & 255u;
                const uint32_t e = min(256u, d_end - (blk << 8));
                n = e - a;
                first_pos = a; last_pos = e - 1u;
                uint32_t docs_[4];
                pk_decode_round<IMP, PK>(seg, blk, lane, docs_, tfv, nr, sbits);
#pragma unroll
                for (int j = 0; j < DE; j++) { ps[j].x = docs_[j]; ps[j].y = sbits[j]; }
                if (n == (uint32_t)(DE * 64)) {
#pragma unroll
                    for (int j = 0; j < DE; j++) {
                        dokm[j] = wballot(ps[j].x <= hi);
                        cnt += (uint32_t)__popcll(dokm[j]);
                    }
                } else {
#pragma unroll
                    for (int j = 0; j < DE; j++) {
                        const uint32_t c0 = (uint32_t)(j * 64);
                        const uint64_t vm = lane_span(a > c0 ? a - c0 : 0u, e > c0 ? min(e - c0, 64u) : 0u);
                        dokm[j] = wballot(ps[j].x <= hi) & vm;
// ... 208 lines not shown
```

### nextsearch-api_amd/csrc/ns_internal.h

```cpp
#pragma once
#include <stdint.h>

namespace ns {

static constexpr uint32_t kTileEmptyBits = 0xFFFFFFFFu;
static constexpr uint32_t kPkBlock = 256;
static constexpr uint32_t kPkStrideDwords = 512;
static constexpr uint32_t kPkTf = 0, kPkNormA = 64, kPkNormB = 128, kPkDoc = 192;
static constexpr uint32_t kSkipDocs = 1024;
static constexpr uint32_t kBmxBlock = 256;

struct DevSeg {
    const uint2* postings;
    const float* pnorm;
    const float* norm;
    const uint2* impacts;
    const uint32_t* packed;
    const uint2* pk_hdr;
    const float* ntab;
    const float* pk_scores;
    const uint32_t* skips;
    const float* blockmax;
    uint64_t     n_postings;
    uint32_t     n_docs;
    uint32_t     n_tiles;
};

struct DevTerm {
    uint64_t list_off;
    uint32_t count;
    float    idf;
    float    weight;
    uint32_t seg;
    uint32_t skip;
    uint32_t bmx;
};

struct DevShare {
    uint32_t first;
    uint32_t count;
    float    idf;
    uint32_t seg;
    uint32_t before;
};

struct DevItem {
    uint64_t bounds_off;
    uint32_t query;
    uint32_t seg;
    uint32_t term_begin;
    uint32_t term_count;
    uint32_t tile_begin;
    uint32_t tile_end;
    uint32_t out_slot;
    uint32_t pad;
};

struct DevWItem {
    uint32_t query;
    uint32_t seg;
    uint32_t term_begin;
    uint32_t term_count;
    uint32_t doc_lo;
    uint32_t doc_hi;
    uint32_t out_slot;
    uint32_t whole;
};

struct DevRItem {
    DevWItem it;
    uint32_t row;
    uint32_t dterm;
};
static constexpr uint32_t kRowLen = 64;

struct DevGroup {
    uint64_t bounds_off;
    uint32_t term_begin;
    uint32_t term_count;
    uint32_t seg;
    uint32_t pad;
};

struct DevQuery {
    uint32_t part_begin;
    uint32_t part_count;
};
constexpr bool merge_is_wide(uint32_t part_count, uint32_t K) { return part_count > 64 && part_count >= K; }

#ifndef NS_WIN_SLACK_THIN
#define NS_WIN_SLACK_THIN 1
#endif
#ifndef NS_WIN_SLACK_GEN
#define NS_WIN_SLACK_GEN 3
#endif
static constexpr uint32_t kWinSlackThin = NS_WIN_SLACK_THIN, kWinSlackGen = NS_WIN_SLACK_GEN;
#if defined(__HIPCC__) || defined(__CUDACC__)
#define NS_HD __host__ __device__
#else
#define NS_HD
#endif
NS_HD inline uint32_t foreign_slack(uint32_t c, uint32_t FB, uint32_t nact, uint32_t Rf) {
    if (Rf <= FB - nact) return 1u;
    if (2u * c * nact > FB) return 1u;
    return c;
}
NS_HD inline float foreign_scale(uint32_t c_eff, uint32_t FB, uint32_t nact, float rcp_Rf) {
    return (float)((int)FB - (int)(c_eff * nact)) * rcp_Rf;
}
NS_HD inline uint32_t foreign_window(uint32_t rem, uint32_t c_eff, float scale) {
    const uint32_t w = c_eff + (uint32_t)((float)rem * scale);
    return (w < rem) ? w : rem;
}

struct Hit {
    float    score;
    uint32_t seg;
    uint32_t doc;
};

}
```

### nextsearch-api_amd/csrc/ns_plan.hpp

```cpp
#pragma once
#include <algorithm>
#include <cmath>
#include <cstdarg>
#include <cstdio>
#include <cstring>
#include <functional>
#include <map>
#include <memory>
#include <string>
#include <thread>
#include <unordered_map>
#include <vector>

#include "../../include/nextsearch_hip.h"
#include "ns_forkjoin.hpp"
#include "ns_internal.h"

namespace ns {

struct VariantDesc { uint32_t hb; uint32_t nt, spt, u; uint32_t d; };
static const VariantDesc kVariants[] = {
    {512, 512, 12, 4, 0},
    {0, 1024, 12, 4, 0},
    {0, 512, 12, 4, 0},
    {0, 256, 16, 4, 0},
    {0, 512, 16, 8, 0},
    {0, 0, 0, 0, 0},
    {0, 0, 0, 0, 0}, {0, 0, 0, 0, 0}, {0, 0, 0, 0, 0}, {0, 0, 0, 0, 0}, {0, 0, 0, 0, 0}, {0, 0, 0, 0, 0},
    {512, 512, 12, 4, 0},
    {256, 512, 12, 4, 0},
    {1024, 512, 12, 4, 0},
    {512, 512, 12, 4, 0},
    {512, 512, 12, 4, 0},
    {1024, 512, 12, 4, 0},
    {512, 512, 12, 4, 1},
    {1024, 512, 12, 4, 1},
    {2048, 512, 12, 4, 1},
};
static constexpr uint32_t kNumVariants = sizeof(kVariants) / sizeof(kVariants[0]);
static constexpr uint32_t kWaveMaxTerms = 64;
static constexpr uint32_t kDefaultSplitPostings = 32768;
static constexpr uint32_t kSplitWorkSmallK = 98304, kSplitWorkLargeK = 131072;
static constexpr uint64_t kWorkForeign = 8, kWorkTile = 2, kWorkMerge = 4;
static constexpr uint32_t kSkipMinCount = 64;
static constexpr uint64_t kItemTermGeneral = 4000, kItemTermThin = 3000, kItemTermTile = 8000;
static constexpr uint32_t kRowMinUsers = 4, kRowCellPostings = 65536;
static constexpr uint32_t kRowMaxTerms = 16;

inline std::string vformat(const char* fmt, va_list ap) {
    char buf[512];
    std::vsnprintf(buf, sizeof(buf), fmt, ap);
    return buf;
}

template <class V>
class ListTable {
public:
    bool empty() const { return n_ == 0; }
    size_t slot_of(uint64_t key) const { return (size_t)((key * 0x9E3779B97F4A7C15ull) >> 20) & (slots_.size() - 1); }
    void prefetch(uint64_t key) const { if (!slots_.empty()) __builtin_prefetch(&slots_[slot_of(key)]); }
    const V* find(uint64_t key) const {
        if (slots_.empty()) return nullptr;
        for (size_t h = slot_of(key);; h = (h + 1) & (slots_.size() - 1)) {
            if (slots_[h].key == key) return &slots_[h].v;
            if (slots_[h].key == kFree) return nullptr;
        }
    }
    V& insert(uint64_t key, bool* fresh) {
        if (2 * n_ >= slots_.size()) rebuild(std::max<size_t>(16, slots_.size() * 2));
        for (size_t h = slot_of(key);; h = (h + 1) & (slots_.size() - 1)) {
            Slot& s = slots_[h];
            if (s.key == key) { *fresh = false; return s.v; }
            if (s.key == kFree) { s.key = key; n_++; *fresh = true; return s.v; }
        }
    }
    void put(uint64_t key, const V& v) { bool fresh; insert(key, &fresh) = v; }
    template <class F> void for_each(F fn) { for (Slot& s : slots_) if (s.key != kFree) fn(s.key, s.v); }
    template <class F> void erase_if(F pred) { refill(slots_.size(), pred); }
    void clear() { slots_.clear(); n_ = 0; }

private:
    static constexpr uint64_t kFree = ~0ull;
    struct Slot { uint64_t key = kFree; V v{}; };
    void rebuild(size_t cap) { refill(cap, [](uint64_t, const V&) { return false; }); }
    template <class F> void refill(size_t cap, F drop) {
        std::vector<Slot> old(cap);
        old.swap(slots_);
        n_ = 0;
        for (const Slot& s : old) if (s.key != kFree && !drop(s.key, s.v)) put(s.key, s.v);
    }
    std::vector<Slot> slots_;
    size_t n_ = 0;
};

struct SegLists {
    struct Imp { uint32_t count, idf_bits; };
    struct Skip { uint32_t count, entry; };
    struct Bmx { uint32_t count, idf_bits, entry; };
    ListTable<Imp> imp;
    ListTable<Skip> skip;
    ListTable<Bmx> bmx;
    std::map<uint32_t, uint32_t> share_lists;
    bool share_admit(uint32_t first, uint32_t count) {
        auto it = share_lists.lower_bound(first);
        if (it != share_lists.end() && (it->first == first ? it->second != count : (uint64_t)first + count > it->first)) return false;
        if (it != share_lists.begin() && (it == share_lists.end() || it->first != first)) {
            auto pv = std::prev(it);
            if ((uint64_t)pv->first + pv->second > first) return false;
        }
        share_lists.emplace(first, count);
        return true;
    }
    bool imp_has(uint32_t first, uint32_t count, uint32_t idf_bits) const {
        const Imp* e = imp.find(first);
        return e && e->count == count && e->idf_bits == idf_bits;
    }
    uint32_t skip_of(uint32_t first, uint32_t count) const {
        const Skip* e = skip.find(first);
        return e && e->count == count ? e->entry + 1u : 0u;
    }
    uint32_t bmx_of(uint32_t first, uint32_t count, uint32_t idf_bits) const {
        const Bmx* e = bmx.find(first);
        return e && e->count == count && e->idf_bits == idf_bits ? e->entry + 1u : 0u;
    }
};

struct SegView {
    uint32_t n_docs = 0, n_tiles = 0;
    uint64_t n_postings = 0;
    bool norm_safe = false;
    bool packed = false;
    SegLists* lists = nullptr;
};

struct ShareRegistry {
    struct Ent { uint32_t count, idf_bits, epoch; bool bad; };
    ListTable<Ent> tab;
    uint32_t epoch = 0;
    uint32_t live = 0;
};

struct PlanSettings {
    uint32_t variant = 0;
    uint32_t min_items = 0;
    uint32_t split_postings = 0;
    int n_cus = 0;
    bool use_impacts = true;
    int use_packed = 1;
    bool use_skips = true;
    bool use_merge = true;
    uint32_t merge_ratio = 8;
    bool use_pruning = false;
    int share_mode = 1;
    uint32_t share_ratio = 48;
    uint64_t share_min_postings = 4u << 20;
    unsigned prep_threads = 0;
    int order_mode = 1, order_coarse = 3;
    bool order_coarse_forced = false;
    uint32_t key_pct[4] = {100, 100, 100, 100};
    uint32_t tile_dens64 = 16;
    int row_mode = 0;
    uint32_t row_min_users = kRowMinUsers;
    uint32_t row_cell_postings = kRowCellPostings;
};

inline size_t place_at(size_t& off, size_t bytes) {
    const size_t o = off;
    off = (off + std::max<size_t>(bytes, 1) + 255) & ~(size_t)255;
    return o;
}


struct HostGroup { DevGroup g; uint32_t query; uint64_t cost; uint64_t cmax; uint64_t work; bool wave; uint8_t cls; bool fast_div; bool signed_in; bool grid; bool merge2;
                   uint32_t rkey1; };

struct RowKey {
    uint32_t seg, first, count, idf_bits, w_bits;
    bool operator==(const RowKey& o) const { return seg == o.seg && first == o.first && count == o.count && idf_bits == o.idf_bits && w_bits == o.w_bits; }
};
struct RowKeyHash {
    size_t operator()(const RowKey& k) const {
        uint64_t h = ((uint64_t)k.seg << 32 | k.first) * 0x9E3779B97F4A7C15ull;
        h ^= ((uint64_t)k.idf_bits << 32 | k.w_bits) * 0xC2B2AE3D27D4EB4Full;
        return (size_t)(h ^ (h >> 29));
    }
};
struct RowKeyEnt { RowKey key; uint32_t users, skip, cells, prod_begin, rank; bool on; };
struct RowCand { uint32_t group, dterm, skip, key; };

constexpr uint32_t kOrderBuckets = 2048;
inline uint32_t order_bucket(uint64_t c) {
    if (c < 32) return kOrderBuckets - 1 - (uint32_t)c;
    const int b = 63 - __builtin_clzll(c);
    const uint32_t key = (uint32_t)b * 32u + (uint32_t)((c >> (b - 5)) & 31u);
    return kOrderBuckets - 1 - std::min(key, kOrderBuckets - 1);
}

struct PrepSlice {
    uint32_t q0 = 0, q1 = 0;
    std::vector<DevTerm> dterms;
    std::vector<HostGroup> groups;
    std::vector<uint32_t> qgroup_begin;
    std::vector<uint32_t> seg_ids;
    std::vector<RowCand> rcand;
    uint64_t bounds_total = 0, postings_total = 0, total_work = 0;
    bool all_imp = true, all_pk = true, any_pruned = false;
    int err_code = NS_OK;
    uint32_t err_query = 0xFFFFFFFFu;
    std::string err_msg;
    std::vector<DevWItem> witems;
    std::vector<uint16_t> wbucket;
    std::vector<uint32_t> wshare;
    std::vector<DevRItem> ritems;
    std::vector<uint16_t> rbucket;
    std::vector<DevItem> items;
    std::vector<uint64_t> item_cost;
    std::vector<DevGroup> bgroups;
    uint32_t n_rows = 0;
    bool direct = true;
    std::vector<uint32_t> hist;
    uint32_t term_off = 0, row_off = 0, bgroup_off = 0;
    uint64_t bounds_off = 0;
    std::vector<uint32_t> start;
    void reset(uint32_t a, uint32_t b) {
        q0 = a; q1 = b;
        dterms.clear(); groups.clear(); qgroup_begin.clear(); seg_ids.clear(); rcand.clear();
        bounds_total = postings_total = total_work = 0; all_imp = true; all_pk = true; any_pruned = false;
        err_code = NS_OK; err_query = 0xFFFFFFFFu; err_msg.clear();
        witems.clear(); wbucket.clear(); wshare.clear(); ritems.clear(); rbucket.clear(); items.clear(); item_cost.clear(); bgroups.clear();
        n_rows = 0; direct = true;
        hist.assign(3 * kOrderBuckets, 0u);
        start.assign(3 * kOrderBuckets, 0u);
        term_off = row_off = bgroup_off = 0; bounds_off = 0;
    }
    void fail_at(uint32_t q, int code, const char* fmt, ...) {
        if (err_code != NS_OK) return;
        va_list ap;
        va_start(ap, fmt);
        err_msg = vformat(fmt, ap);
        va_end(ap);
        err_code = code; err_query = q;
    }
};

struct BatchPlan {
    std::string err;
    uint32_t n_dterms = 0, n_rows = 0, n_witems = 0, n_items = 0, n_bgroups = 0;
    uint32_t n_class[3] = {0, 0, 0};
    uint64_t bounds_total = 0, postings_total = 0;
    bool direct = false;
    bool all_imp = false, all_pk = false, pruned = false;
    bool shared = false;
    std::vector<DevShare> share_build;
    uint64_t share_postings = 0;
    std::vector<uint32_t> wide_q;
    uint32_t n_ritems = 0, n_pitems = 0, n_pterms = 0;
    std::vector<RowKeyEnt> rkeys;
    std::vector<DevWItem> pitems;
    std::vector<DevTerm> pterms;
    struct Layout { size_t items, witems, terms, groups, queries, segs, wideq, share, ritems, pitems, rstats, bytes; } layout{};
    bool deal = false;
    uint32_t deal_shift = 0;
    std::vector<uint32_t> bucket_pos;

    const PlanSettings* cfg = nullptr;
    const std::vector<SegView>* segs = nullptr;
    const ns_query_desc* queries = nullptr;
    const ns_term_ref* terms = nullptr;
    uint32_t n_queries = 0, k = 0, flags = 0;
    bool auto_mode = false, want_imp = false, row_try = false;
    unsigned width = 1;
// ... 18 lines not shown
    void fork(const std::function<void(unsigned)>& fn) {
        if (width == 1) fn(0); else pool->run(width, fn);
    }

    int group(const PlanSettings& C, const std::vector<SegView>& SV, ShareRegistry& reg, const ns_query_desc* queries_,
              const ns_term_ref* terms_, uint32_t n_queries_, uint32_t k_, uint32_t flags_) {
        cfg = &C; segs = &SV; queries = queries_; terms = terms_; n_queries = n_queries_; k = k_; flags = flags_;
        const bool wave_path = kVariants[C.variant].hb != 0;
        auto_mode = C.variant == 0;

        width = 1;
        if (n_queries >= 3000 && C.prep_threads != 1) {
            unsigned want = C.prep_threads ? C.prep_threads : std::min<unsigned>(std::max(1u, std::thread::hardware_concurrency()), 8u);
            uint64_t n_refs = 0;
            for (uint32_t q = 0; q < n_queries; q++) n_refs += queries[q].term_count;
            width = std::max(1u, std::min<unsigned>(want, std::max<unsigned>(n_queries / 1500, (unsigned)std::min<uint64_t>(n_refs / 6000, 64))));
        }
        if (width > 1 && (!pool || pool->width() < width)) pool.reset(new ForkJoin(width));
        if (slices.size() < width) slices.resize(width);
        for (unsigned s = 0; s < width; s++) slices[s].reset((uint32_t)((uint64_t)n_queries * s / width), (uint32_t)((uint64_t)n_queries * (s + 1) / width));
        want_imp = C.use_impacts && auto_mode;
        row_try = want_imp && C.row_mode != 0 && C.share_mode != 0 && C.use_skips && !(flags & NS_FLAG_AND) && k <= 32;

        fork([&](unsigned si) {
            PrepSlice& S = slices[si];
            S.all_imp = want_imp;
            S.qgroup_begin.reserve(S.q1 - S.q0 + 1);
            for (uint32_t q = S.q0; q < S.q1; q++) {
                S.qgroup_begin.push_back((uint32_t)S.groups.size());
                const ns_query_desc qd = queries[q];
                if (qd.term_count && !terms) { S.fail_at(q, NS_E_INVAL, "terms is NULL"); break; }
                S.seg_ids.clear();
                bool bad = false;
                for (uint32_t i = 0; i < qd.term_count && !bad; i++) {
                    const ns_term_ref& r = terms[qd.term_begin + i];
                    if (r.seg_id >= SV.size() || !SV[r.seg_id].lists) { S.fail_at(q, NS_E_INVAL, "query %u term %u: unknown segment %u", q, i, r.seg_id); bad = true; break; }
                    const SegView& s = SV[r.seg_id];
                    if (r.byte_off % 8 != 0) { S.fail_at(q, NS_E_INVAL, "query %u term %u: byte_off %llu not a multiple of 8", q, i, (unsigned long long)r.byte_off); bad = true; break; }
                    if (r.byte_off / 8 + r.count > s.n_postings) { S.fail_at(q, NS_E_INVAL, "query %u term %u: list [%llu,+%u) outside segment %u (%llu postings)", q, i, (unsigned long long)(r.byte_off / 8), r.count, r.seg_id, (unsigned long long)s.n_postings); bad = true; break; }
                    if (std::find(S.seg_ids.begin(), S.seg_ids.end(), r.seg_id) == S.seg_ids.end()) S.seg_ids.push_back(r.seg_id);
                }
                if (bad) break;
                std::sort(S.seg_ids.begin(), S.seg_ids.end());
                for (uint32_t sid : S.seg_ids) {
                    const SegView& sv = SV[sid];
                    HostGroup hg{};
                    hg.fast_div = sv.norm_safe;
                    if (!sv.packed) S.all_pk = false;
                    hg.g.term_begin = (uint32_t)S.dterms.size();
                    hg.g.seg = sid;
                    hg.query = q;
                    for (uint32_t i = 0; i < qd.term_count; i++) {
                        const ns_term_ref& r = terms[qd.term_begin + i];
                        if (r.seg_id != sid) continue;
                        DevTerm t{};
                        t.list_off = r.byte_off / 8;
                        t.count = r.count;
                        t.idf = r.idf;
                        t.weight = r.qweight;
                        t.seg = sid;
                        S.dterms.push_back(t);
                        hg.cost += r.count;
                        hg.cmax = std::max<uint64_t>(hg.cmax, r.count);
                        if (S.all_imp) {
                            uint32_t ib; std::memcpy(&ib, &r.idf, 4);
                            S.all_imp = sv.lists->imp_has((uint32_t)(r.byte_off / 8), r.count, ib);
                        }
                        if (!(r.idf >= 9.313225746154785e-10f && r.idf <= 1073741824.0f)) hg.fast_div = false;
                        if (std::signbit(r.idf) || std::signbit(r.qweight)) hg.signed_in = true;
                    }
                    hg.g.term_count = (uint32_t)S.dterms.size() - hg.g.term_begin;
                    if ((flags & NS_FLAG_AND) && hg.g.term_count > 255) { S.fail_at(q, NS_E_INVAL, "AND mode supports at most 255 term refs per (query, segment)"); bad = true; break; }
                    hg.wave = wave_path && hg.g.term_count <= kWaveMaxTerms;
                    {
                        const uint64_t rest = hg.cost - hg.cmax;
                        const uint32_t nd = std::max<uint32_t>(sv.n_docs, 1);
                        if (rest * 32 <= hg.cmax) hg.cls = 1;
                        else if (hg.g.term_count >= 2 && hg.cost * 64 >= (uint64_t)nd * C.tile_dens64) hg.cls = 2;
                        else hg.cls = 0;
                        hg.work = !auto_mode ? hg.cost : (hg.cls == 2 ? hg.cost * kWorkTile : hg.cmax + rest * kWorkForeign);
                        hg.merge2 = auto_mode && C.use_merge && hg.cls == 0 && hg.g.term_count == 2 && rest * C.merge_ratio >= hg.cmax;
                        if (hg.merge2) hg.work = hg.cmax + rest * kWorkMerge;
                    }
                    if (row_try && hg.wave && hg.cls == 1 && !hg.signed_in && hg.g.term_count <= kRowMaxTerms && hg.cmax >= kSkipMinCount &&
                        sv.n_docs > 0 && !sv.lists->skip.empty() && !(C.use_pruning && hg.g.term_count == 1)) {
                        const DevTerm* dt = S.dterms.data() + hg.g.term_begin;
                        uint32_t d = 0;
                        while (dt[d].count != hg.cmax) d++;
                        const uint32_t sk = sv.lists->skip_of((uint32_t)dt[d].list_off, dt[d].count);
                        if (sk) S.rcand.push_back(RowCand{(uint32_t)S.groups.size(), d, sk, 0u});
                    }
                    if (!hg.wave) {
                        hg.g.bounds_off = S.bounds_total;
                        S.bounds_total += (uint64_t)(sv.n_tiles + 1) * hg.g.term_count;
                    }
                    S.postings_total += hg.cost;
                    S.total_work += hg.work;
                    S.groups.push_back(hg);
                }
                if (bad) break;
            }
            S.qgroup_begin.resize(S.q1 - S.q0 + 1, (uint32_t)S.groups.size());
        });
        {
            const PrepSlice* first = nullptr;
            for (unsigned s = 0; s < width; s++)
                if (slices[s].err_code != NS_OK && (!first || slices[s].err_query < first->err_query)) first = &slices[s];
            if (first) return failed(first->err_code, "%s", first->err_msg.c_str());
        }
        bounds_total = postings_total = total_work = 0;
        n_dterms = G = 0;
        all_imp = want_imp; all_pk = C.use_packed != 0 && auto_mode;
        for (unsigned s = 0; s < width; s++) {
            PrepSlice& S = slices[s];
            S.term_off = n_dterms; S.bounds_off = bounds_total;
            n_dterms += (uint32_t)S.dterms.size(); G += (uint32_t)S.groups.size();
            bounds_total += S.bounds_total; postings_total += S.postings_total; total_work += S.total_work;
            all_imp = all_imp && S.all_imp;
            all_pk = all_pk && S.all_pk;
        }
        if (bounds_total >= (1ull << 32)) return failed(NS_E_INVAL, "batch too large: %llu boundary entries; split the batch", (unsigned long long)bounds_total);

        share_build.clear();
        share_postings = 0;
        shared = false;
        if (!all_imp && want_imp && C.share_mode != 0 && !all_pk && postings_total > 0 &&
            (C.share_mode == 2 || postings_total >= C.share_min_postings)) {
            shared = true;
            if (++reg.epoch == 0) {
                reg.tab.for_each([](uint64_t, ShareRegistry::Ent& en) { en.epoch = 0; });
                reg.epoch = 1;
            }
            const uint32_t epoch = reg.epoch;
            for (unsigned sl = 0; sl < width && shared; sl++) {
                const std::vector<DevTerm>& dts = slices[sl].dterms;
                for (size_t ti = 0; ti < dts.size(); ti++) {
                    if (ti + 8 < dts.size()) reg.tab.prefetch(((uint64_t)dts[ti + 8].seg << 32) | (uint32_t)dts[ti + 8].list_off);
                    const DevTerm& t = dts[ti];
                    if (!t.count) continue;
                    SegLists* sg = SV[t.seg].lists;
                    uint32_t ib; std::memcpy(&ib, &t.idf, 4);
                    const uint32_t first = (uint32_t)t.list_off;
                    if (!sg->imp.empty()) {
                        if (sg->imp_has(first, t.count, ib)) continue;
                        shared = false; break;
                    }
                    bool fresh = false;
                    ShareRegistry::Ent& en = reg.tab.insert(((uint64_t)t.seg << 32) | first, &fresh);
                    if (fresh) { en.count = t.count; en.idf_bits = ib; en.epoch = 0; en.bad = !sg->share_admit(first, t.count); }
                    if (en.bad || en.count != t.count) { shared = false; break; }
                    if (en.idf_bits != ib) {
                        if (reg.live || en.epoch == epoch) { shared = false; break; }
                        en.idf_bits = ib;
                    }
                    if (en.epoch != epoch) {
                        en.epoch = epoch;
                        if (share_postings + t.count >= (1ull << 32)) { shared = false; break; }
                        share_build.push_back(DevShare{first, t.count, t.idf, t.seg, (uint32_t)share_postings});
                        share_postings += t.count;
                        if (C.share_mode == 1 && share_postings * C.share_ratio > postings_total) { shared = false; break; }
                    }
                }
            }
            if (shared && C.share_mode == 1 && postings_total < (uint64_t)C.share_ratio * share_postings) shared = false;
        }
        return NS_OK;
    }

    static void row_cell(uint32_t n_docs, uint32_t cells, uint32_t i, uint32_t& lo, uint32_t& hi) {
        lo = (uint32_t)((uint64_t)n_docs * i / cells);
        hi = (uint32_t)((uint64_t)n_docs * (i + 1) / cells);
        lo -= lo % kSkipDocs;
        if (i + 1 < cells) hi -= hi % kSkipDocs;
    }

    int cut() {
        const PlanSettings& C = *cfg;
        const std::vector<SegView>& SV = *segs;
        if (shared) all_imp = true;
        else { share_build.clear(); share_postings = 0; }

        const uint32_t min_items = C.min_items ? C.min_items : (uint32_t)std::max(C.n_cus, 1) * 24u;
        int small_mode = 0;
        uint64_t split_postings = C.split_postings ? C.split_postings
                                  : (!auto_mode ? kDefaultSplitPostings : (k <= 32 ? kSplitWorkSmallK : kSplitWorkLargeK));
        bool fine_cut = false;
        if (!C.split_postings && auto_mode) {
            const uint64_t fine = total_work / ((uint64_t)std::max(C.n_cus, 1) * 96u);
            fine_cut = fine < split_postings;
            split_postings = std::min<uint64_t>(split_postings, std::max<uint64_t>(fine, 16384));
            const uint64_t per_slot = total_work / ((uint64_t)std::max(C.n_cus, 1) * 24u);
            small_mode = per_slot >= 2 * split_postings ? 0 : (per_slot >= split_postings ? 1 : 2);
        }
        uint32_t chunks_per_group = 1;
        if (G > 0 && G < min_items) chunks_per_group = std::min<uint32_t>((min_items + G - 1) / G, 1024u);
        dq.assign(n_queries, DevQuery{});

        rkeys.clear(); pitems.clear(); pterms.clear();
        n_ritems = n_pitems = n_pterms = 0;
        if (shared && row_try) {
            std::unordered_map<RowKey, uint32_t, RowKeyHash> index;
            for (unsigned s = 0; s < width; s++) {
                PrepSlice& S = slices[s];
                for (RowCand& c : S.rcand) {
                    const DevTerm& t = S.dterms[S.groups[c.group].g.term_begin + c.dterm];
                    RowKey key{t.seg, (uint32_t)t.list_off, t.count, 0u, 0u};
                    std::memcpy(&key.idf_bits, &t.idf, 4); std::memcpy(&key.w_bits, &t.weight, 4);
                    auto ins = index.emplace(key, (uint32_t)rkeys.size());
                    if (ins.second) rkeys.push_back(RowKeyEnt{key, 0u, c.skip, 0u, 0u, 0u, false});
                    c.key = ins.first->second;
                    rkeys[c.key].users++;
                }
            }
            for (RowKeyEnt& e : rkeys) {
                if (C.row_mode != 2 && e.users < C.row_min_users) continue;
                const SegView& sg = SV[e.key.seg];
                uint32_t cells = 1;
                while ((uint64_t)cells * std::max<uint32_t>(C.row_cell_postings, 1u) < e.key.count && cells * 2 <= sg.n_docs / kSkipDocs && cells < 4096) cells <<= 1;
                e.on = true; e.cells = cells; e.prod_begin = n_pitems; e.rank = n_pterms++;
                DevTerm t{};
                t.list_off = e.key.first; t.count = e.key.count; t.seg = e.key.seg; t.skip = e.skip;
                std::memcpy(&t.idf, &e.key.idf_bits, 4); std::memcpy(&t.weight, &e.key.w_bits, 4);
                pterms.push_back(t);
                for (uint32_t i = 0; i < cells; i++) {
                    DevWItem it{};
                    it.seg = e.key.seg;
                    it.term_begin = n_dterms + e.rank;
                    it.term_count = 1;
                    row_cell(sg.n_docs, cells, i, it.doc_lo, it.doc_hi);
                    it.out_slot = n_pitems++;
                    it.whole = (cells == 1 ? 1u : 0u) | 4u | 64u;
                    pitems.push_back(it);
                }
            }
            for (unsigned s = 0; s < width; s++) {
                PrepSlice& S = slices[s];
                for (const RowCand& c : S.rcand)
                    if (rkeys[c.key].on) S.groups[c.group].rkey1 = c.key + 1u;
            }
        }

        fork([&](unsigned si) {
            PrepSlice& S = slices[si];
            for (uint32_t q = S.q0; q < S.q1; q++) {
                dq[q].part_begin = S.n_rows;
                for (uint32_t gi = S.qgroup_begin[q - S.q0]; gi < S.qgroup_begin[q - S.q0 + 1]; gi++) {
                    HostGroup& hg = S.groups[gi];
                    hg.g.term_begin += S.term_off;
                    const SegView& sg = SV[hg.g.seg];
                    if (sg.n_docs == 0) continue;
                    if (hg.wave) {
                        DevTerm* dt = S.dterms.data() + (hg.g.term_begin - S.term_off);
                        uint64_t sp_ = (auto_mode && hg.cls != 0) ? split_postings * 2 : split_postings;
                        if (auto_mode && hg.cls != 0 && small_mode) sp_ = small_mode == 2 ? split_postings / 2 : split_postings;
                        const uint64_t want = std::max<uint64_t>((hg.work + sp_ - 1) / sp_, chunks_per_group);
                        uint32_t ns = (uint32_t)std::min<uint64_t>(std::max<uint64_t>(want, 1), std::min<uint32_t>(sg.n_docs, 4096));
                        if (auto_mode && ns > 1) {
                            uint32_t p2 = 1;
                            while (p2 < ns) p2 <<= 1;
                            if (!small_mode && (uint64_t)ns * ns * 2 < (uint64_t)p2 * p2) p2 >>= 1;
                            if (k > 32 && p2 < 8) p2 = 8;
                            ns = std::min<uint32_t>(p2, std::min<uint32_t>(sg.n_docs, 4096));
                        }
                        const RowKeyEnt* rk = hg.rkey1 ? &rkeys[hg.rkey1 - 1u] : nullptr;
                        if (rk) ns = rk->cells;
                        if (auto_mode && C.use_skips && (hg.cls == 2 || ns > 1 || rk) && !sg.lists->skip.empty()) {
                            for (uint32_t ti = 0; ti < hg.g.term_count; ti++) {
                                if (dt[ti].count < kSkipMinCount) continue;
                                dt[ti].skip = sg.lists->skip_of((uint32_t)dt[ti].list_off, dt[ti].count);
                                if (dt[ti].skip) hg.grid = true;
                            }
                        }
                        bool pruned_ = false;
                        if (auto_mode && C.use_pruning && hg.g.term_count == 1 && !sg.lists->bmx.empty()) {
                            uint32_t ib; std::memcpy(&ib, &dt[0].idf, 4);
                            if (dt[0].idf > 0.0f && std::isfinite(dt[0].idf) && dt[0].weight > 0.0f && std::isfinite(dt[0].weight)) {
                                dt[0].bmx = sg.lists->bmx_of((uint32_t)dt[0].list_off, dt[0].count, ib);
                                pruned_ = dt[0].bmx != 0;
                            }
                            if (pruned_) S.any_pruned = true;
                        }
                        const uint64_t per_term = hg.cls == 2 ? kItemTermTile : (hg.cls == 1 ? kItemTermThin : kItemTermGeneral);
                        uint64_t key = hg.work / ns + 1 + (auto_mode ? per_term * hg.g.term_count : 0);
                        if (fine_cut && hg.cls == 0) key = key * 5 / 8;
                        else if (auto_mode && k > 32 && hg.cls == 0) key = key * 3 / 4;
                        if (auto_mode) key = key * C.key_pct[hg.merge2 ? 3 : hg.cls] / 100;
                        if (rk) key = (hg.cost - hg.cmax) * kWorkForeign / ns + 1 + kItemTermThin * hg.g.term_count;
                        const bool wide = auto_mode && hg.g.term_count > 16;
                        const uint32_t bucket = order_bucket(key);
                        uint64_t big_off = 0;
                        for (uint32_t ti = 0, cm = 0; ti < hg.g.term_count; ti++)
                            if (dt[ti].count >= cm) { cm = dt[ti].count; big_off = dt[ti].list_off; }
                        for (uint32_t i = 0; i < ns; i++) {
                            DevWItem it{};
                            it.query = q;
                            it.seg = hg.g.seg;
                            it.term_begin = hg.g.term_begin;
                            it.term_count = hg.g.term_count;
                            it.doc_lo = (uint32_t)((uint64_t)sg.n_docs * i / ns);
                            it.doc_hi = (uint32_t)((uint64_t)sg.n_docs * (i + 1) / ns);
                            if (hg.grid) {
                                it.doc_lo -= it.doc_lo % kSkipDocs;
                                if (i + 1 < ns) it.doc_hi -= it.doc_hi % kSkipDocs;
                            }
                            if (rk) row_cell(sg.n_docs, ns, i, it.doc_lo, it.doc_hi);
                            if (it.doc_hi <= it.doc_lo) continue;
                            it.out_slot = S.n_rows++;
                            it.whole = (ns == 1 ? 1u : 0u) | (hg.fast_div ? 8u : 0u) | (hg.signed_in ? 16u : 0u) | (hg.grid ? (hg.cls == 2 ? 32u : 64u) : 0u);
                            if (auto_mode) it.whole |= (hg.cls == 2 ? 2u : 0u) | (hg.cls == 1 ? 4u : 0u) | (pruned_ ? 128u : 0u) | (hg.merge2 && hg.wave ? 256u : 0u);
                            if (rk) {
                                uint32_t d = 0;
                                while (dt[d].count != hg.cmax) d++;
                                S.ritems.push_back(DevRItem{it, rk->prod_begin + i, d});
                                S.rbucket.push_back((uint16_t)bucket);
                                S.hist[2 * kOrderBuckets + bucket]++;
                                continue;
                            }
                            S.witems.push_back(it);
                            S.wbucket.push_back((uint16_t)(bucket | (wide ? 0x8000u : 0u)));
                            {
                                uint64_t h = big_off * 0x9E3779B97F4A7C15ull;
                                h ^= h >> 29;
                                const uint32_t r12 = (uint32_t)(((uint64_t)it.doc_lo << 12) / std::max<uint32_t>(sg.n_docs, 1u)) & 4095u;
                                S.wshare.push_back(((it.seg & 63u) << 26) | (r12 << 14) | (uint32_t)((h >> 40) & 0x3FFFu));
                            }
                            S.hist[(wide ? kOrderBuckets : 0) + bucket]++;
                        }
                    } else {
                        DevGroup g = hg.g;
                        g.bounds_off += S.bounds_off;
                        S.bgroups.push_back(g);
                        const uint32_t nt = sg.n_tiles;
                        const uint32_t chunks = std::min(chunks_per_group, nt);
                        const uint32_t per = (nt + chunks - 1) / chunks;
                        for (uint32_t tb = 0; tb < nt; tb += per) {
                            DevItem it{};
                            it.bounds_off = g.bounds_off;
                            it.query = q;
                            it.seg = g.seg;
                            it.term_begin = g.term_begin;
                            it.term_count = g.term_count;
                            it.tile_begin = tb;
                            it.tile_end = std::min(nt, tb + per);
                            it.out_slot = S.n_rows++;
                            S.item_cost.push_back(hg.cost * (it.tile_end - it.tile_begin) / nt + 1);
                            S.items.push_back(it);
                        }
                    }
                }
                dq[q].part_count = S.n_rows - dq[q].part_begin;
                if (dq[q].part_count != 1) S.direct = false;
            }
        });
        n_rows = n_witems = n_items = n_bgroups = 0;
        direct = n_queries > 0;
        pruned = false;
        for (unsigned s = 0; s < width; s++) {
            PrepSlice& S = slices[s];
            S.row_off = n_rows; S.bgroup_off = n_bgroups;
            n_rows += S.n_rows; n_witems += (uint32_t)S.witems.size(); n_ritems += (uint32_t)S.ritems.size(); n_items += (uint32_t)S.items.size(); n_bgroups += (uint32_t)S.bgroups.size();
            direct = direct && S.direct;
            pruned = pruned || S.any_pruned;
        }
        n_class[0] = n_class[1] = n_class[2] = 0;
        {
            uint32_t pos = 0;
            bucket_pos.assign(kOrderBuckets + 1, 0u);
            for (uint32_t half = 0; half < 2; half++) {
                for (uint32_t bkt = 0; bkt < kOrderBuckets; bkt++) {
                    if (half == 0) bucket_pos[bkt] = pos;
                    for (unsigned s = 0; s < width; s++) {
                        slices[s].start[half * kOrderBuckets + bkt] = pos;
                        pos += slices[s].hist[half * kOrderBuckets + bkt];
                    }
                }
                if (half == 0) { n_class[0] = pos; bucket_pos[kOrderBuckets] = pos; }
            }
            n_class[1] = pos - n_class[0];
            if (pos != n_witems) return failed(NS_E_STATE, "internal: launch order holds %u of %u work items", pos, n_witems);
            if (!auto_mode) { n_class[0] = n_class[1] = 0; }
            uint32_t rpos = 0;
            for (uint32_t bkt = 0; bkt < kOrderBuckets; bkt++)
                for (unsigned s = 0; s < width; s++) {
                    slices[s].start[2 * kOrderBuckets + bkt] = rpos;
                    rpos += slices[s].hist[2 * kOrderBuckets + bkt];
                }
            if (rpos != n_ritems) return failed(NS_E_STATE, "internal: launch order holds %u of %u row consumers", rpos, n_ritems);
        }
        sorted_items.clear();
        if (n_items) {
            struct Cost { uint64_t c; uint32_t slice, idx; };
            std::vector<Cost> ic;
            ic.reserve(n_items);
            for (unsigned s = 0; s < width; s++)
                for (uint32_t i = 0; i < slices[s].items.size(); i++) ic.push_back({slices[s].item_cost[i], s, i});
            std::stable_sort(ic.begin(), ic.end(), [](const Cost& a, const Cost& b) { return a.c > b.c; });
// ... 113 lines not shown
```

### nextsearch-api_amd/csrc/ns_row_kernel.hip

```cpp
#pragma once
#include <hip/hip_runtime.h>
#include <stdint.h>

#include "ns_driver_kernel.hip"

namespace ns {

template <int HK, int CB, int TMAX>
__global__ void __launch_bounds__(64) __attribute__((amdgpu_waves_per_eu(6, 8))) k_rscore(const DevRItem* __restrict__ items, uint32_t n_items,
                                                const DevTerm* __restrict__ terms, const DevSeg* __restrict__ segs,
                                                const Hit* __restrict__ row_hits, const uint32_t* __restrict__ row_nhits,
                                                Hit* __restrict__ out_hits, uint32_t* __restrict__ out_nhits,
                                                uint64_t* __restrict__ out_found, uint32_t K, uint32_t* __restrict__ stats) {
    __shared__ __attribute__((aligned(16))) uint32_t s_tbl[2 * HK];
    __shared__ __attribute__((aligned(16))) float s_vals[64];
    __shared__ __attribute__((aligned(16))) uint8_t s_mcnt[16];
    __shared__ uint64_t s_cand[CB];
    __shared__ __attribute__((aligned(16))) uint4 s_tab[TMAX];
    __shared__ uint32_t s_aux[TMAX];
    const int lane = threadIdx.x & 63;
    const uint32_t item_idx = blockIdx.x;
    if (item_idx >= n_items) return;
    const DevRItem ri = items[item_idx];
    DevWItem it = ri.it;
    it.whole &= 121u;
    RowArgs ra;
    ra.hits = row_hits + (size_t)ri.row * kRowLen;
    ra.nhits = row_nhits[ri.row];
    ra.dterm = ri.dterm;
    ra.stats = stats;
    if (dscore_body<HK / 2, 64, false, CB, true, 0, true>(it, terms, segs, s_tbl, s_vals, s_mcnt, s_cand, s_tab, s_aux, out_hits, out_nhits,
                                                          out_found, K, lane, ra))
        return;
    if (lane == 0) atomicAdd(stats, 1u);
    wave_sync();
    dscore_body<HK / 2, 64, false, CB, true, 0, false>(it, terms, segs, s_tbl, s_vals, s_mcnt, s_cand, s_tab, s_aux, out_hits, out_nhits,
                                                       out_found, K, lane);
}

}
```

### nextsearch-api_amd/csrc/ns_wave_kernel.hip

```cpp
#pragma once
#include <hip/hip_runtime.h>
#include <stdint.h>

#include "ns_internal.h"

namespace ns {

__device__ __forceinline__ void wave_sync() {
    __builtin_amdgcn_fence(__ATOMIC_RELEASE, "wavefront");
    __builtin_amdgcn_wave_barrier();
    __builtin_amdgcn_fence(__ATOMIC_ACQUIRE, "wavefront");
}

__device__ __forceinline__ uint32_t rdlane(uint32_t v, uint32_t l) { return (uint32_t)__builtin_amdgcn_readlane((int)v, (int)l); }
__device__ __forceinline__ uint32_t lanes_below(unsigned long long mask) {
    return __builtin_amdgcn_mbcnt_hi((uint32_t)(mask >> 32), __builtin_amdgcn_mbcnt_lo((uint32_t)mask, 0u));
}

template <int M>
__device__ __forceinline__ uint32_t lane_xor_u32(uint32_t v, int lane) {
    if constexpr (M == 1) return (uint32_t)__builtin_amdgcn_update_dpp(0, (int)v, 0xB1, 0xf, 0xf, true);
    else if constexpr (M == 2) return (uint32_t)__builtin_amdgcn_update_dpp(0, (int)v, 0x4E, 0xf, 0xf, true);
    else if constexpr (M < 32) return (uint32_t)__builtin_amdgcn_ds_swizzle((int)v, (M << 10) | 0x1F);
    else return (uint32_t)__builtin_amdgcn_ds_bpermute((lane ^ 32) << 2, (int)v);
// ... 215 lines not shown
            const ns_f2 a2 = {a[j], a[j + 1]}, b2 = {b[j], b[j + 1]};
            const ns_f2 q2 = ns_div_short2(a2, b2);
            q[j] = q2.x; q[j + 1] = q2.y;
        }
        if (N & 1) q[N - 1] = ns_div_short(a[N - 1], b[N - 1]);
    } else {
#pragma unroll
        for (int j = 0; j < N; j++) q[j] = a[j] / b[j];
    }
}

__device__ __forceinline__ uint32_t list_lower_bound(const uint2* lst, uint32_t count, uint32_t doc) {
    uint32_t lo = 0, hi = count;
    while (lo < hi) {
        uint32_t mid = lo + ((hi - lo) >> 1);
        if (lst[mid].x < doc) lo = mid + 1; else hi = mid;
    }
    return lo;
}

__device__ __forceinline__ void list_range(const uint2* lst, uint32_t count, uint32_t doc_lo, uint32_t doc_hi, uint32_t n_docs,
                                           uint32_t& first, uint32_t& last) {
    uint32_t a0 = 0, b0 = count, a1 = 0, b1 = count;
    if (count > 64u && n_docs > 0u) {
        const float dens = (float)count / (float)n_docs;
        const uint32_t margin = 64u + (uint32_t)(8.0f * __builtin_sqrtf((float)count * (1.0f - (dens < 1.0f ? dens : 1.0f)) + 1.0f));
        const uint32_t g0 = min(count, (uint32_t)((float)doc_lo * dens)), g1 = min(count, (uint32_t)((float)doc_hi * dens));
        const uint32_t l0 = g0 > margin ? g0 - margin : 0u, h0 = min(count - 1u, g0 + margin);
        const uint32_t l1 = g1 > margin ? g1 - margin : 0u, h1 = min(count - 1u, g1 + margin);
        const uint32_t vl0 = lst[l0].x, vh0 = lst[h0].x, vl1 = lst[l1].x, vh1 = lst[h1].x;
        if (vl0 < doc_lo) a0 = l0 + 1u;
        if (vh0 >= doc_lo) b0 = h0;
        if (vl1 < doc_hi) a1 = l1 + 1u;
        if (vh1 >= doc_hi) b1 = h1;
        if (a0 > b0) { a0 = 0; b0 = count; }
        if (a1 > b1) { a1 = 0; b1 = count; }
    }
    while (a0 < b0 || a1 < b1) {
        const uint32_t m0 = a0 + ((b0 - a0) >> 1), m1 = a1 + ((b1 - a1) >> 1);
        const uint32_t v0 = lst[min(m0, count - 1u)].x, v1 = lst[min(m1, count - 1u)].x;
        if (a0 < b0) { if (v0 < doc_lo) a0 = m0 + 1u; else b0 = m0; }
        if (a1 < b1) { if (v1 < doc_hi) a1 = m1 + 1u; else b1 = m1; }
    }
    first = a0;
    last = a1;
}

template <int CTRL, int ROWMASK>
__device__ __forceinline__ uint32_t dpp_mov(uint32_t old, uint32_t src) {
    return (uint32_t)__builtin_amdgcn_update_dpp((int)old, (int)src, CTRL, ROWMASK, 0xf, false);
}
__device__ __forceinline__ uint32_t wave_min_dpp(uint32_t v) {
    v = min(v, dpp_mov<0x111, 0xf>(0xFFFFFFFFu, v));
    v = min(v, dpp_mov<0x112, 0xf>(0xFFFFFFFFu, v));
    v = min(v, dpp_mov<0x114, 0xf>(0xFFFFFFFFu, v));
    v = min(v, dpp_mov<0x118, 0xf>(0xFFFFFFFFu, v));
    v = min(v, dpp_mov<0x142, 0xa>(0xFFFFFFFFu, v));
    v = min(v, dpp_mov<0x143, 0xc>(0xFFFFFFFFu, v));
    return rdlane(v, 63);
}
__device__ __forceinline__ uint32_t wave_max_dpp(uint32_t v) {
    v = max(v, dpp_mov<0x111, 0xf>(0u, v));
    v = max(v, dpp_mov<0x112, 0xf>(0u, v));
    v = max(v, dpp_mov<0x114, 0xf>(0u, v));
    v = max(v, dpp_mov<0x118, 0xf>(0u, v));
    v = max(v, dpp_mov<0x142, 0xa>(0u, v));
    v = max(v, dpp_mov<0x143, 0xc>(0u, v));
    return rdlane(v, 63);
}
__device__ __forceinline__ uint32_t wave_incl_scan_dpp(uint32_t v) {
    v += dpp_mov<0x111, 0xf>(0u, v);
    v += dpp_mov<0x112, 0xf>(0u, v);
    v += dpp_mov<0x114, 0xf>(0u, v);
    v += dpp_mov<0x118, 0xf>(0u, v);
    v += dpp_mov<0x142, 0xa>(0u, v);
    v += dpp_mov<0x143, 0xc>(0u, v);
    return v;
}

typedef unsigned int nat_u2 __attribute__((ext_vector_type(2)));
typedef const __attribute__((address_space(1))) nat_u2* gp_u2;
typedef const __attribute__((address_space(1))) float* gp_f32;
typedef const __attribute__((address_space(1))) uint32_t* gp_u32;

__device__ __forceinline__ uint2 item_list_range(const DevWItem& it, const DevSeg& seg, const DevTerm& tm) {
    uint32_t cur = 0, end = tm.count;
    if (!(it.whole & 1u)) {
        if ((it.whole & 64u) && tm.skip != 0u) {
            const gp_u32 sk = (gp_u32)seg.skips + (tm.skip - 1u);
            cur = sk[it.doc_lo / kSkipDocs] - (uint32_t)tm.list_off;
            end = sk[(it.doc_hi + (kSkipDocs - 1u)) / kSkipDocs] - (uint32_t)tm.list_off;
        } else {
            list_range(seg.postings + tm.list_off, tm.count, it.doc_lo, it.doc_hi, seg.n_docs, cur, end);
        }
        if (end < cur) end = cur;
    }
    return make_uint2(cur, end);
}

__global__ void k_pnorm(const uint2* __restrict__ postings, const float* __restrict__ norm, float* __restrict__ pnorm,
                        uint64_t n_postings, uint32_t n_docs) {
    uint64_t i = (uint64_t)blockIdx.x * blockDim.x + threadIdx.x;
    const uint64_t stride = (uint64_t)gridDim.x * blockDim.x;
    for (; i < n_postings; i += stride) {
        uint32_t d = postings[i].x;
        pnorm[i] = d < n_docs ? norm[d] : 1.0f;
    }
}

__global__ void __launch_bounds__(64) k_pack(const uint2* __restrict__ postings, const uint16_t* __restrict__ nidx,
                                             uint32_t* __restrict__ packed, uint2* __restrict__ hdr, uint64_t n_postings,
                                             uint32_t n_docs, uint32_t n_blocks) {
    const uint32_t b = blockIdx.x;
    if (b >= n_blocks) return;
    const uint32_t lane = threadIdx.x;
    uint32_t doc[4], tf[4], ni[4];
    uint32_t mn = 0xFFFFFFFFu, mx = 0u;
#pragma unroll
    for (int c = 0; c < 4; c++) {
        const uint64_t g = (uint64_t)b * kPkBlock + (uint32_t)c * 64u + lane;
        doc[c] = 0xFFFFFFFFu; tf[c] = 0; ni[c] = 0;
        if (g < n_postings) {
            const uint2 p = postings[g];
            doc[c] = p.x; tf[c] = p.y;
            ni[c] = p.x < n_docs ? nidx[p.x] : 0u;
            mn = min(mn, p.x); mx = max(mx, p.x);
        }
    }
    mn = wave_min_dpp(mn);
    mx = wave_max_dpp(mx);
    if (mn > mx) { mn = 0; mx = 0; }
    const uint32_t span = mx - mn;
    const uint32_t code = span < 256u ? 0u : (span < 65536u ? 1u : 2u);
    const uint32_t base = code == 2u ? 0u : mn;
    uint32_t* blk = packed + (uint64_t)b * kPkStrideDwords;
    uint32_t off[4];
#pragma unroll
    for (int c = 0; c < 4; c++) off[c] = doc[c] == 0xFFFFFFFFu ? 0u : doc[c] - base;
    blk[kPkTf + lane] = min(tf[0], 255u) | (min(tf[1], 255u) << 8) | (min(tf[2], 255u) << 16) | (min(tf[3], 255u) << 24);
    blk[kPkNormA + lane] = ni[0] | (ni[1] << 16);
    blk[kPkNormB + lane] = ni[2] | (ni[3] << 16);
    if (code == 0u) {
        blk[kPkDoc + lane] = off[0] | (off[1] << 8) | (off[2] << 16) | (off[3] << 24);
    } else if (code == 1u) {
        blk[kPkDoc + lane] = off[0] | (off[1] << 16);
        blk[kPkDoc + 64 + lane] = off[2] | (off[3] << 16);
    } else {
#pragma unroll
        for (int c = 0; c < 4; c++) blk[kPkDoc + c * 64 + lane] = doc[c];
    }
    if (lane == 0) hdr[b] = make_uint2(base, code);
}

}
```

### nextsearch-api_amd/nsbind.py

```python
import ctypes as C
import os

import numpy as np

HERE = os.path.dirname(os.path.abspath(__file__))
HIP_LIB_PATH = os.environ.get("NS_HIP_LIB") or os.path.join(HERE, "libnextsearch_hip.so")
HOST_LIB_PATH = os.path.join(HERE, "libnextsearch_host.so")

NS_OK = 0
NS_FLAG_OR = 0
NS_FLAG_AND = 1
NS_SORT_DESC, NS_SORT_ASC = 0, 0x1000
NS_ROLE_SHOULD, NS_ROLE_MUST, NS_ROLE_NOT = 0, 1, 2
NS_INFO_IMPACTS = 0x100
NS_INFO_PACKED = 0x200
NS_INFO_PRUNED = 0x400
NS_INFO_SHARED = 0x800
NS_MAX_K = 100


class NsTermRef(C.Structure):
    _fields_ = [("seg_id", C.c_uint32), ("count", C.c_uint32), ("byte_off", C.c_uint64),
                ("idf", C.c_float), ("qweight", C.c_float)]


class NsQueryDesc(C.Structure):
    _fields_ = [("term_begin", C.c_uint32), ("term_count", C.c_uint32)]


class NsHit(C.Structure):
    _fields_ = [("score", C.c_float), ("seg_id", C.c_uint32), ("doc_id", C.c_uint32)]


class NsBatchInfo(C.Structure):
    _fields_ = [("postings", C.c_uint64), ("algo_bytes", C.c_uint64), ("n_queries", C.c_uint32),
                ("n_items", C.c_uint32), ("n_term_refs", C.c_uint32), ("tile_docs", C.c_uint32),
                ("k", C.c_uint32), ("flags", C.c_uint32), ("last_score_kernel_ms", C.c_float),
                ("last_total_ms", C.c_float), ("timed_runs", C.c_uint32), ("shared_lists", C.c_uint32),
                ("sum_score_kernel_ms", C.c_double), ("sum_total_ms", C.c_double), ("shared_postings", C.c_uint64)]


HIT_DTYPE = np.dtype([("score", "<f4"), ("seg", "<u4"), ("doc", "<u4")])
TERM_DTYPE = np.dtype([("seg_id", "<u4"), ("count", "<u4"), ("byte_off", "<u8"), ("idf", "<f4"), ("qweight", "<f4")])
QDESC_DTYPE = np.dtype([("term_begin", "<u4"), ("term_count", "<u4")])
assert HIT_DTYPE.itemsize == C.sizeof(NsHit) == 12
assert TERM_DTYPE.itemsize == C.sizeof(NsTermRef) == 24
assert QDESC_DTYPE.itemsize == C.sizeof(NsQueryDesc) == 8
PAGE_CURSOR_DTYPE = np.dtype([("set", "<u4"), ("rank", "<u4"), ("seg", "<u4"), ("doc", "<u4")])
PAGE_MODES = {"or": 0, "and": 1, "boolean": 2, "sorted": 3, "boolean_sorted": 4}
CURSOR_DTYPE = np.dtype([("rank", "<u4"), ("seg", "<u4"), ("doc", "<u4"), ("set", "<u4")])

HIP_SYMBOLS = [
    "ns_facet_upload", "ns_facet_release", "ns_facet_count", "ns_facet_tile_docs",
    "ns_dockeys_upload", "ns_dockeys_release", "ns_search_sorted", "ns_sorted_kernel_ms",
    "ns_search_boolean", "ns_boolean_kernel_ms", "ns_search_boolean_after", "ns_search_sorted_after",
    "ns_facet_count_boolean", "ns_search_sorted_boolean", "ns_boolean_sets_kernel_ms",
    "ns_segment_filter",
    "ns_ctx_create", "ns_ctx_destroy", "ns_ctx_set_stream", "ns_last_error", "ns_device_name",
    "ns_segment_upload", "ns_segment_release", "ns_segment_upload_begin", "ns_segment_upload_append", "ns_segment_upload_end", "ns_search_batch", "ns_batch_prepare",
    "ns_batch_bind_outputs", "ns_batch_run", "ns_batch_stream", "ns_batch_gap_ms", "ns_batch_sync", "ns_batch_fetch", "ns_batch_get_info",
    "ns_batch_destroy", "ns_set_tuning", "ns_segment_build_impacts", "ns_ctx_use_impacts", "ns_ctx_set_host_threads", "ns_ctx_set_overlap", "ns_segment_build_packed", "ns_ctx_use_packed", "ns_segment_build_skips", "ns_ctx_use_skips", "ns_segment_build_blockmax", "ns_ctx_use_pruning", "ns_ctx_use_merge", "ns_ctx_share_scores", "ns_ctx_share_rows", "ns_batch_row_stats",
    "ns_invert_forward", "ns_segment_upload_inverted", "ns_merge_rank_rows", "ns_sem_upload", "ns_sem_release", "ns_sem_topk",
    "ns_ac_upload", "ns_ac_suggest", "ns_ac_release", "ns_ac_build_fuzzy", "ns_ac_fuzzy", "ns_ac_fuzzy_prefix",
    "ns_forward_build", "ns_forward_get_info", "ns_forward_fetch", "ns_forward_destroy",
    "ns_forward_merge", "ns_forward_invert", "ns_compact_doc_cut", "ns_ctx_use_docsort",
    "ns_forward_merge_keep",
    "ns_docterms_upload", "ns_docterms_select", "ns_docterms_destroy", "ns_docterms_doc_cut",
]
HOST_SYMBOLS = [
    "nsh_parse_boolean", "nsh_engine_search_boolean_batch", "nsh_engine_search_boolean_json",
    "nsh_parse_cursor", "nsh_cursor_text", "nsh_engine_search_after_batch", "nsh_engine_search_boolean_after_batch", "nsh_engine_search_sorted_after_batch",
    "nsh_engine_search_page_json",
    "nsh_engine_facet_boolean_batch", "nsh_engine_search_boolean_sorted_batch", "nsh_engine_search_boolean_faceted_json", "nsh_engine_search_boolean_sorted_json",
    "nsh_engine_sort_keys", "nsh_engine_search_sorted_batch", "nsh_engine_search_sorted_json", "nsh_engine_release_sorted", "nsh_engine_sort_tables_on_device",
    "nsh_engine_facet_buckets", "nsh_engine_facet_batch", "nsh_engine_search_faceted_json", "nsh_engine_release_facets", "nsh_engine_facet_tables_on_device",
    "nsh_date_key", "nsh_engine_filter_bits", "nsh_engine_open_filter", "nsh_engine_open_filter_bits", "nsh_engine_close_filter", "nsh_engine_open_filters",
    "nsh_engine_search_filtered_batch", "nsh_engine_search_filtered_json",
    "nsh_gen_index", "nsh_engine_open", "nsh_engine_open_multi", "nsh_engine_num_devices", "nsh_shard_bounds", "nsh_engine_close", "nsh_engine_reload", "nsh_engine_error", "nsh_engine_ctx",
    "nsh_engine_num_segments", "nsh_engine_segment_name", "nsh_engine_segment_info",
    "nsh_engine_segment_doc_len", "nsh_engine_segment_postings", "nsh_engine_lookup", "nsh_bm25_idf",
    "nsh_base_terms", "nsh_engine_build_refs", "nsh_engine_search_json", "nsh_free",
    "nsh_engine_search_batch", "nsh_engine_prepare", "nsh_engine_doc_metadata", "nsh_engine_hits_to_json", "nsh_engine_search_batch_json",
    "nsh_engine_build_impacts", "nsh_engine_use_impacts", "nsh_engine_build_packed", "nsh_engine_use_packed", "nsh_engine_build_blockmax", "nsh_engine_use_pruning", "nsh_engine_use_merge", "nsh_engine_share_scores", "nsh_engine_use_skips", "nsh_invert_segment", "nsh_invert_error",
    "nsh_engine_semantic_info", "nsh_engine_expand", "nsh_engine_semantic_row", "nsh_engine_set_cache", "nsh_engine_cache_size",
    "nsh_engine_suggest_json", "nsh_engine_suggest_batch", "nsh_engine_suggest_table", "nsh_suggest_split", "nsh_suggest_clamp_limit",
    "nsh_engine_correct_batch", "nsh_engine_did_you_mean_json", "nsh_correct_auto_edits", "nsh_engine_correct_build_ms",
    "nsh_engine_complete_batch", "nsh_engine_complete_json",
    "nsh_index_documents", "nsh_index_error", "nsh_engine_open_noload", "nsh_engine_add_documents",
    "nsh_merge_segments", "nsh_compact_error", "nsh_engine_compact",
    "nsh_engine_find_documents", "nsh_engine_delete_documents", "nsh_engine_delete_by_id",
    "nsh_similar_select_host", "nsh_similar_clamp_terms", "nsh_similar_clamp_k", "nsh_similar_qweight", "nsh_similar_defaults",
    "nsh_engine_similar_term_stats", "nsh_engine_similar_batch", "nsh_engine_more_like_this_json", "nsh_engine_release_similar",
    "nsh_engine_similar_segments_on_device",
]

class NsForwardInfo(C.Structure):
    _fields_ = [("struct_size", C.c_uint32), ("kept_docs", C.c_uint32), ("n_terms", C.c_uint32), ("n_docs", C.c_uint32),
                ("n_pairs", C.c_uint64), ("term_bytes", C.c_uint64), ("n_tokens", C.c_uint64), ("kept_tokens", C.c_uint64),
                ("device_bytes", C.c_uint64), ("device_ms", C.c_float), ("pad", C.c_uint32)]


class NshIndexStats(C.Structure):
    _fields_ = [("struct_size", C.c_uint32), ("n_docs_in", C.c_uint32), ("n_docs", C.c_uint32), ("n_terms", C.c_uint32),
                ("text_bytes", C.c_uint64), ("tokens", C.c_uint64), ("kept_tokens", C.c_uint64), ("pairs", C.c_uint64),
                ("device_bytes", C.c_uint64), ("avgdl", C.c_float), ("device_ms", C.c_float), ("call_s", C.c_double), ("total_s", C.c_double)]

    def as_dict(self):
        return {k: getattr(self, k) for k, _ in self._fields_ if k != "struct_size"}


class NsForwardSrc(C.Structure):
    _fields_ = [("n_docs", C.c_uint32), ("doc_len", C.c_void_p), ("counts", C.c_void_p), ("n_pairs", C.c_uint64), ("pairs", C.c_void_p),
                ("n_terms", C.c_uint32), ("term_bytes", C.c_void_p), ("term_offsets", C.c_void_p)]


class NshCompactStats(C.Structure):
    _fields_ = [("struct_size", C.c_uint32), ("sources", C.c_uint32), ("n_docs", C.c_uint32), ("n_terms", C.c_uint32),
                ("terms_in", C.c_uint64), ("pairs", C.c_uint64), ("device_bytes", C.c_uint64),
                ("merge_ms", C.c_float), ("invert_ms", C.c_float), ("call_s", C.c_double), ("total_s", C.c_double)]

    def as_dict(self):
        return {k: getattr(self, k) for k, _ in self._fields_ if k != "struct_size"}


class NshDeleteStats(C.Structure):
    _fields_ = [("struct_size", C.c_uint32), ("segments_rewritten", C.c_uint32), ("segments_dropped", C.c_uint32), ("docs_deleted", C.c_uint32),
                ("uids_not_found", C.c_uint32), ("terms_dropped", C.c_uint32),
                ("pairs_in", C.c_uint64), ("pairs_out", C.c_uint64), ("device_bytes", C.c_uint64),
                ("merge_ms", C.c_float), ("invert_ms", C.c_float), ("call_s", C.c_double), ("total_s", C.c_double)]

    def as_dict(self):
        return {k: getattr(self, k) for k, _ in self._fields_ if k != "struct_size"}


class NshFacetSpec(C.Structure):
    _fields_ = [("kind", C.c_uint32), ("n_custom_labels", C.c_uint32), ("custom_buckets", C.c_void_p), ("n_custom", C.c_uint64),
                ("custom_labels", C.POINTER(C.c_char_p))]


FACET_KINDS = {"year": 0, "month": 1, "custom": 2}


class NshSortSpec(C.Structure):
    _fields_ = [("kind", C.c_uint32), ("ascending", C.c_uint32), ("custom_keys", C.c_void_p), ("n_custom", C.c_uint64)]


SORT_ORDERS = {"newest": (0, 0), "oldest": (0, 1)}

_hip = None
_host = None


def hip_lib():
    global _hip
    if _hip is None:
        if not os.path.exists(HIP_LIB_PATH):
            raise RuntimeError(f"{HIP_LIB_PATH} is missing: build it with `make -C nextsearch-api_amd` "
                               "(there is no fallback path)")
        L = C.CDLL(HIP_LIB_PATH, mode=C.RTLD_GLOBAL)
        vp, u32, u64, i32 = C.c_void_p, C.c_uint32, C.c_uint64, C.c_int
        L.ns_ctx_create.argtypes = [i32, C.POINTER(vp)]
        L.ns_ctx_destroy.argtypes = [vp]
        L.ns_ctx_destroy.restype = None
        L.ns_ctx_set_stream.argtypes = [vp, vp]
        L.ns_ac_upload.argtypes = [vp, vp, vp, vp, u32, C.POINTER(vp)]
        L.ns_ac_suggest.argtypes = [vp, vp, vp, vp, u32, u32, vp, vp, C.POINTER(C.c_float)]
        L.ns_ac_release.argtypes = [vp, vp]
        L.ns_ac_build_fuzzy.argtypes = [vp, vp, C.POINTER(C.c_float)]
        L.ns_ac_fuzzy.argtypes = [vp, vp, vp, vp, u32, vp, u32, u32, vp, vp, vp, C.POINTER(C.c_float)]
        L.ns_ac_fuzzy_prefix.argtypes = [vp, vp, vp, vp, u32, vp, u32, u32, vp, vp, vp, C.POINTER(C.c_float)]
        L.ns_last_error.argtypes = [vp]
        L.ns_last_error.restype = C.c_char_p
        L.ns_device_name.argtypes = [vp]
        L.ns_device_name.restype = C.c_char_p
        L.ns_segment_upload.argtypes = [vp, u32, u32, C.c_float, vp, vp, u64, C.POINTER(vp)]
        L.ns_segment_release.argtypes = [vp, vp]
        L.ns_segment_upload_begin.argtypes = [vp, u32, u32, C.c_float, vp, u64, C.POINTER(vp)]
        L.ns_segment_upload_append.argtypes = [vp, vp, vp, u64]
        L.ns_segment_upload_end.argtypes = [vp, vp]
        L.ns_segment_build_impacts.argtypes = [vp, vp, vp, vp, vp, u32]
        L.ns_ctx_use_impacts.argtypes = [vp, i32]
        L.ns_segment_build_skips.argtypes = [vp, vp, vp, vp, u32]
        L.ns_ctx_use_skips.argtypes = [vp, i32]
        L.ns_segment_filter.argtypes = [vp, vp, u32, vp, vp, vp, u32, vp, vp, vp, C.POINTER(u64), C.POINTER(C.c_float), C.POINTER(vp)]
        L.ns_ctx_set_host_threads.argtypes = [vp, u32]
        L.ns_ctx_set_overlap.argtypes = [vp, i32]
        L.ns_segment_build_packed.argtypes = [vp, vp]
        L.ns_ctx_use_packed.argtypes = [vp, i32]
        L.ns_segment_build_blockmax.argtypes = [vp, vp, vp, vp, vp, u32]
        L.ns_ctx_use_pruning.argtypes = [vp, i32]
        L.ns_ctx_use_merge.argtypes = [vp, i32]
        L.ns_ctx_share_scores.argtypes = [vp, i32]
        if hasattr(L, "ns_ctx_share_rows"):
            L.ns_ctx_share_rows.argtypes = [vp, i32]
            L.ns_batch_row_stats.argtypes = [vp, vp]
        L.ns_sem_upload.argtypes = [vp, vp, u32, u32, C.POINTER(vp)]
        L.ns_sem_release.argtypes = [vp, vp]
        L.ns_sem_topk.argtypes = [vp, vp, vp, u32, u32, C.c_float, vp, vp, vp, vp, vp, vp]
        L.ns_merge_rank_rows.argtypes = [vp, vp, vp, vp, u32, u32, u32, vp, u32, vp, vp, vp]
        L.ns_invert_forward.argtypes = [vp, vp, u32, vp, u64, u32, vp, vp, C.POINTER(u64), vp]
        L.ns_segment_upload_inverted.argtypes = [vp, vp, vp, vp, u64, u32, vp, vp, C.POINTER(u64), vp]
        L.ns_search_batch.argtypes = [vp, vp, vp, u32, u32, vp, vp, vp, u32]
        L.ns_batch_prepare.argtypes = [vp, vp, vp, u32, u32, u32, C.POINTER(vp)]
        L.ns_batch_bind_outputs.argtypes = [vp, vp, vp, vp]
        L.ns_batch_run.argtypes = [vp, i32]
        L.ns_batch_gap_ms.argtypes = [vp, vp, C.POINTER(C.c_float)]
        L.ns_batch_stream.argtypes = [vp]
        L.ns_batch_stream.restype = vp
        L.ns_batch_sync.argtypes = [vp]
        L.ns_batch_fetch.argtypes = [vp, vp, vp, vp]
        L.ns_batch_get_info.argtypes = [vp, C.POINTER(NsBatchInfo)]
        L.ns_batch_destroy.argtypes = [vp]
        L.ns_batch_destroy.restype = None
        L.ns_set_tuning.argtypes = [vp, u32, u32, u32]
        L.ns_forward_build.argtypes = [vp, vp, u64, vp, u32, C.POINTER(vp)]
        L.ns_forward_get_info.argtypes = [vp, C.POINTER(NsForwardInfo)]
        L.ns_forward_fetch.argtypes = [vp, vp, vp, vp, vp, vp, vp]
        L.ns_forward_destroy.argtypes = [vp]
        L.ns_forward_destroy.restype = None
        L.ns_forward_merge.argtypes = [vp, vp, u32, C.POINTER(vp)]
        L.ns_forward_invert.argtypes = [vp, vp, vp, C.POINTER(u64), vp]
        L.ns_compact_doc_cut.argtypes = []
        L.ns_compact_doc_cut.restype = u32
        L.ns_ctx_use_docsort.argtypes = [vp, i32]
        L.ns_forward_merge_keep.argtypes = [vp, vp, vp, u32, C.POINTER(vp)]
        L.ns_docterms_upload.argtypes = [vp, vp, vp, vp, C.POINTER(vp)]
        L.ns_docterms_select.argtypes = [vp, vp, u32, u32, u32, u32, u32, vp, vp, vp, C.POINTER(C.c_float)]
        L.ns_docterms_destroy.argtypes = [vp]
        L.ns_docterms_destroy.restype = None
        L.ns_docterms_doc_cut.argtypes = []
        L.ns_docterms_doc_cut.restype = u32
        L.ns_facet_upload.argtypes = [vp, u32, vp, u32, C.POINTER(vp)]
        L.ns_facet_release.argtypes = [vp, vp]
        L.ns_facet_count.argtypes = [vp, vp, u32, vp, u32, u32, vp, vp, vp, u32, vp, vp, C.POINTER(C.c_float)]
        L.ns_facet_tile_docs.argtypes = []
        L.ns_facet_tile_docs.restype = u32
        L.ns_dockeys_upload.argtypes = [vp, u32, vp, C.POINTER(vp)]
        L.ns_dockeys_release.argtypes = [vp, vp]
        L.ns_search_sorted.argtypes = [vp, vp, u32, vp, u32, u32, u32, vp, vp, vp, u32, vp, vp, vp, vp, C.POINTER(C.c_float)]
        L.ns_sorted_kernel_ms.argtypes = [C.POINTER(C.c_float), i32]
        L.ns_search_boolean.argtypes = [vp, vp, u32, vp, vp, u32, u32, vp, vp, u32, vp, vp, vp, C.POINTER(C.c_float)]
        L.ns_boolean_kernel_ms.argtypes = [C.POINTER(C.c_float), i32]
        L.ns_search_boolean_after.argtypes = [vp, vp, u32, vp, vp, u32, u32, vp, vp, vp, u32, vp, vp, vp, vp, C.POINTER(C.c_float)]
        L.ns_search_sorted_after.argtypes = [vp, vp, u32, vp, u32, u32, u32, vp, vp, vp, vp, u32, vp, vp, vp, vp, vp, C.POINTER(C.c_float)]
        L.ns_facet_count_boolean.argtypes = [vp, vp, u32, vp, vp, u32, vp, vp, vp, u32, vp, vp, C.POINTER(C.c_float)]
        L.ns_search_sorted_boolean.argtypes = [vp, vp, u32, vp, vp, u32, u32, u32, vp, vp, vp, vp, u32, vp, vp, vp, vp, vp, C.POINTER(C.c_float)]
        L.ns_boolean_sets_kernel_ms.argtypes = [C.POINTER(C.c_float), i32]
        for name in DEBUG_COUNTERS:
            if hasattr(L, name):
                getattr(L, name).argtypes = [C.POINTER(u64), i32]
        _hip = L
    return _hip


DEBUG_COUNTERS = {"ns_debug_counters": 32, "ns_debug_tile_counters": 12, "ns_debug_merge_counters": 16, "ns_debug_topk_counters": 4,
                  "ns_debug_join_counters": 16, "ns_debug_facet_counters": 8, "ns_debug_sorted_counters": 9,
                  "ns_debug_boolean_counters": 8, "ns_debug_after_counters": 5, "ns_debug_fuzzy_counters": 17,
                  "ns_debug_boolean_sets_counters": 12}


def debug_counters(reset=False):
    L = hip_lib()
    out = {}
    for name, n in DEBUG_COUNTERS.items():
        if hasattr(L, name):
            buf = (C.c_uint64 * n)()
            if getattr(L, name)(buf, int(bool(reset))) != 0:
                raise RuntimeError(name + " failed")
            out[name] = [int(v) for v in buf]
    return out


def fuzzy_counters(reset=False):
    L = hip_lib()
    if not hasattr(L, "ns_debug_fuzzy_counters"):
        return None
    buf = (C.c_uint64 * DEBUG_COUNTERS["ns_debug_fuzzy_counters"])()
    if L.ns_debug_fuzzy_counters(buf, int(bool(reset))) != 0:
# ... 1628 lines not shown
```

Baseline: 8.976 million.

## Add per-list rank directories for constant-time membership probes in row kernel

```diff
diff --git a/include/nextsearch_hip.h b/include/nextsearch_hip.h
--- a/include/nextsearch_hip.h
+++ b/include/nextsearch_hip.h
@@ -98,6 +98,7 @@
 
 int ns_ctx_share_rows(ns_ctx* ctx, int mode);
 int ns_batch_row_stats(ns_batch* b, uint32_t out[4]);
+uint64_t ns_segment_dir_bytes(const ns_seg* seg);
 
 int ns_search_batch(ns_ctx* ctx, const ns_query_desc* queries, const ns_term_ref* terms,
                     uint32_t n_queries, uint32_t k, ns_hit* hits_out, uint32_t* nhits_out,
diff --git a/nextsearch-api_amd/csrc/ns_api.hip b/nextsearch-api_amd/csrc/ns_api.hip
--- a/nextsearch-api_amd/csrc/ns_api.hip
+++ b/nextsearch-api_amd/csrc/ns_api.hip
@@ -65,6 +65,8 @@
     std::vector<uint32_t*> skip_retired;
     uint64_t skip_cap = 0, skip_used = 0;
     uint32_t skip_entries() const { return (n_docs + kSkipDocs - 1) / kSkipDocs + 2; }
+    uint32_t dir_entries() const { return (n_docs + kDirDocs - 1) / kDirDocs; }
+    uint64_t dir_bytes = 0;
     float* d_blockmax = nullptr;
     std::vector<float*> bmx_retired;
     uint64_t bmx_cap = 0, bmx_used = 0;
@@ -82,6 +84,7 @@
     hipStream_t pull_stream = nullptr;
     bool overlap = false, flip = false;
     hipStream_t row_stream = nullptr;
+    uint32_t dir_min_count = kDirMinCount;
     std::string err;
     std::string devname;
     std::vector<ns_seg*> segs;
@@ -215,6 +218,8 @@
     if (const char* rm = std::getenv("NS_SHARE_ROWS")) ctx->cfg.row_mode = std::max(0, std::min(2, std::atoi(rm)));
     if (const char* ru = std::getenv("NS_ROW_MIN_USERS")) ctx->cfg.row_min_users = (uint32_t)std::max(1, std::atoi(ru));
     if (const char* rc = std::getenv("NS_ROW_CELL")) ctx->cfg.row_cell_postings = (uint32_t)std::max(1, std::atoi(rc));
+    if (const char* rr = std::getenv("NS_ROW_REACH")) ctx->cfg.row_reach = (uint32_t)std::max(1, std::atoi(rr));
+    if (const char* dm = std::getenv("NS_DIR_MIN")) ctx->dir_min_count = (uint32_t)std::max(1, std::atoi(dm));
     {
         const char* rf = std::getenv("NS_ROW_FORK");
         if ((!rf || std::atoi(rf) != 0) && hipStreamCreateWithFlags(&ctx->row_stream, hipStreamNonBlocking) != hipSuccess) { ctx->row_stream = nullptr; (void)hipGetLastError(); }
@@ -315,7 +320,7 @@
     for (float* p : s->bmx_retired) (void)hipFree(p);
     s->bmx_retired.clear();
     s->d_blockmax = nullptr; s->bmx_cap = s->bmx_used = 0; s->lists.bmx.clear();
-    s->d_skips = nullptr; s->skip_cap = s->skip_used = 0; s->lists.skip.clear();
+    s->d_skips = nullptr; s->skip_cap = s->skip_used = 0; s->lists.skip.clear(); s->lists.dir.clear(); s->dir_bytes = 0;
     s->d_postings = nullptr; s->d_norm = nullptr; s->d_pnorm = nullptr; s->d_impacts = nullptr; s->d_packed = nullptr;
     s->d_pk_hdr = nullptr; s->d_pk_scores = nullptr; s->d_nidx = nullptr; s->d_ntab = nullptr;
 }
@@ -704,6 +709,34 @@
     if (b) bad[l] = 1u;
 }
 
+__global__ void __launch_bounds__(256) k_dir_build(const uint2* __restrict__ postings, const uint32_t* __restrict__ sk, uint4* __restrict__ dir,
+                                                   uint32_t first, uint32_t count, uint32_t n_entries) {
+    const uint32_t j = blockIdx.x * 256 + threadIdx.x;
+    if (j >= n_entries) return;
+    const uint32_t d0 = j * kDirDocs, endp = first + count;
+    const uint32_t cell = d0 / kSkipDocs;
+    const uint32_t a = sk[cell];
+    const uint32_t n = min(sk[cell + 1u] - a, kSkipDocs);
+    uint32_t lo = 0, len = n;
+#pragma unroll
+    for (int step = 0; step < 11; step++) {
+        const uint32_t half = len >> 1;
+        const bool below = len > 0u && postings[a + lo + half].x < d0;
+        lo = below ? lo + half + 1u : lo;
+        len = below ? len - half - 1u : half;
+    }
+    const uint32_t p0 = a + lo;
+    uint64_t bits = 0ull;
+#pragma unroll 4
+    for (uint32_t i = 0; i < kDirDocs; i++) {
+        if (p0 + i >= endp) break;
+        const uint32_t d = postings[p0 + i].x;
+        if (d - d0 >= kDirDocs) break;
+        bits |= 1ull << (d - d0);
+    }
+    dir[j] = make_uint4((uint32_t)bits, (uint32_t)(bits >> 32), p0 - first, 0u);
+}
+
 extern "C" int ns_segment_build_skips(ns_ctx* ctx, ns_seg* seg, const uint64_t* byte_off, const uint32_t* counts, uint32_t n_lists) {
     if (!ctx || !seg) return fail(ctx, NS_E_INVAL, "ns_segment_build_skips: null argument");
     if (seg->pending || seg->id >= ctx->segs.size() || ctx->segs[seg->id] != seg) return fail(ctx, NS_E_INVAL, "segment does not belong to this ctx");
@@ -721,7 +754,11 @@
     if (lists.empty()) return NS_OK;
     const uint32_t per_list = seg->skip_entries();
     const size_t n = lists.size();
-    const uint64_t need = seg->skip_used + (uint64_t)n * per_list;
+    const uint32_t dir_floor = std::max(seg->n_docs / kDirDocs, ctx->dir_min_count), dir_dwords = seg->dir_entries() * 4u;
+    size_t n_dirs = 0;
+    for (const auto& l : lists) n_dirs += l.count >= dir_floor ? 1 : 0;
+    const uint64_t dir_base = (seg->skip_used + (uint64_t)n * per_list + 3u) & ~3ull;
+    const uint64_t need = n_dirs ? dir_base + (uint64_t)n_dirs * dir_dwords : seg->skip_used + (uint64_t)n * per_list;
     if (need >= (1ull << 32) - 1) return fail(ctx, NS_E_INVAL, "ns_segment_build_skips: %llu table entries do not fit 32 bits", (unsigned long long)need);
     hipError_t e = hipSuccess;
     if (need > seg->skip_cap) {
@@ -758,9 +795,24 @@
     if (e == hipSuccess) e = hipStreamSynchronize(ctx->stream);
     (void)hipFree(d_tmp);
     if (e != hipSuccess) return fail(ctx, NS_E_HIP, "ns_segment_build_skips: %s", hipGetErrorString(e));
-    for (size_t i = 0; i < n; i++)
-        if (!bad[i] && !seg->lists.skip.find(lists[i].first)) seg->lists.skip.put(lists[i].first, {lists[i].count, (uint32_t)(seg->skip_used + i * per_list)});
+    size_t di = 0;
+    for (size_t i = 0; i < n; i++) {
+        const bool reg = !bad[i] && !seg->lists.skip.find(lists[i].first);
+        if (reg) seg->lists.skip.put(lists[i].first, {lists[i].count, (uint32_t)(seg->skip_used + i * per_list)});
+        if (lists[i].count < dir_floor) continue;
+        const uint64_t at = dir_base + (uint64_t)(di++) * dir_dwords;
+        if (!reg || at / 4 + 1 >= (1ull << (32 - kDirTermBits))) continue;
+        hipLaunchKernelGGL(k_dir_build, dim3((seg->dir_entries() + 255) / 256), dim3(256), 0, ctx->stream, seg->d_postings,
+                           seg->d_skips + seg->skip_used + i * per_list, (uint4*)(seg->d_skips + at), lists[i].first, lists[i].count, seg->dir_entries());
+        seg->lists.dir.put(lists[i].first, {lists[i].count, (uint32_t)(at / 4)});
+        seg->dir_bytes += (uint64_t)dir_dwords * 4;
+    }
     seg->skip_used = need;
+    if (n_dirs) {
+        e = hipGetLastError();
+        if (e == hipSuccess) e = hipStreamSynchronize(ctx->stream);
+        if (e != hipSuccess) { seg->lists.dir.clear(); seg->dir_bytes = 0; return fail(ctx, NS_E_HIP, "ns_segment_build_skips: rank directories: %s", hipGetErrorString(e)); }
+    }
     return NS_OK;
 }
 
@@ -1469,6 +1521,17 @@
     info->sum_score_kernel_ms = b->sum_score_ms;
     info->sum_total_ms = b->sum_total_ms;
     return NS_OK;
+}
+
+extern "C" uint64_t ns_segment_dir_bytes(const ns_seg* seg) { return seg ? seg->dir_bytes : 0; }
+
+extern "C" long long ns_debug_read_dir(ns_seg* seg, uint64_t list_off, void* out, uint32_t cap) {
+    if (!seg || (cap && !out)) return NS_E_INVAL;
+    const SegLists::Dir* d = list_off < (1ull << 32) ? seg->lists.dir.find((uint32_t)list_off) : nullptr;
+    if (!d || !seg->d_skips) return 0;
+    const uint32_t n = seg->dir_entries();
+    if (std::min(n, cap) && hipMemcpy(out, seg->d_skips + (uint64_t)d->entry * 4, (size_t)std::min(n, cap) * 16, hipMemcpyDeviceToHost) != hipSuccess) return -1;
+    return n;
 }
 
 extern "C" int ns_batch_row_stats(ns_batch* b, uint32_t out[4]) {
diff --git a/nextsearch-api_amd/csrc/ns_driver_kernel.hip b/nextsearch-api_amd/csrc/ns_driver_kernel.hip
--- a/nextsearch-api_amd/csrc/ns_driver_kernel.hip
+++ b/nextsearch-api_amd/csrc/ns_driver_kernel.hip
@@ -75,7 +75,7 @@
     return upto_hi & ~upto_lo;
 }
 
-struct RowArgs { const Hit* hits; uint32_t nhits; uint32_t dterm; uint32_t* stats; };
+struct RowArgs { const Hit* hits; uint32_t nhits; uint32_t dterm; uint32_t* stats; uint32_t dir; };
 
 template <int NB, int FB, bool AND, int CB = 256, bool IMP = false, int PK = 0, bool ROW = false>
 __device__ __forceinline__ bool dscore_body(const DevWItem& it, const DevTerm* __restrict__ terms, const DevSeg* __restrict__ segs,
@@ -165,6 +165,8 @@
     uint64_t r_left = 0ull;
     bool row_complete = false;
     gp_u32 d_skips = nullptr;
+    gp_u4 d_dir = nullptr;
+    uint32_t d_first = 0;
     if constexpr (ROW) {
         const uint32_t nrow = min(ra.nhits, kRowLen);
         const Hit rh = ra.hits[lane];
@@ -173,6 +175,9 @@
         found_s = d_end - d_cur;
         row_complete = nrow == d_end - d_cur;
         d_skips = (gp_u32)seg.skips + (terms[it.term_begin + dl].skip - 1u);
+        const uint32_t dir1 = (uint32_t)__builtin_amdgcn_readfirstlane((int)ra.dir);
+        if (dir1) d_dir = (gp_u4)seg.skips + (dir1 - 1u);
+        d_first = rdlane(base, dl);
         NS_CNT(19, 1);
     }
 
@@ -458,31 +463,40 @@
                 static_assert(FE == 1, "one foreign posting per lane");
                 const bool own = fmine[0];
                 const uint32_t doc = own ? fdoc[0] : lo;
-                const uint32_t cell = doc / kSkipDocs;
-                uint32_t a = d_skips[cell];
-                uint32_t n = d_skips[cell + 1u] - a;
                 bool hit = false;
                 uint32_t hbits = 0u;
-#pragma unroll
-                for (int step = 0; step < 4; step++) {
-                    const uint32_t s8 = (n + 7u) >> 3;
-                    nat_u2 pv[7];
-#pragma unroll
-                    for (int i = 0; i < 7; i++) {
-                        const uint32_t e = (uint32_t)(i + 1) * s8;
-                        pv[i] = stream[a + ((e <= n && e != 0u) ? e - 1u : 0u)];
-                    }
-                    uint32_t c = 0u;
-#pragma unroll
-                    for (int i = 0; i < 7; i++) {
-                        const uint32_t e = (uint32_t)(i + 1) * s8;
-                        const bool valid = e <= n && e != 0u;
-                        c += (valid && pv[i].x < doc) ? 1u : 0u;
-                        if (valid && pv[i].x == doc) { hit = true; hbits = pv[i].y; }
-                    }
-                    const bool closed = c < 7u && (c + 1u) * s8 <= n;
-                    a += c * s8;
-                    n = (n == 0u) ? 0u : (closed ? s8 - 1u : n - c * s8);
+                if (d_dir != nullptr) {
+                    const nat_u4 e = d_dir[doc / kDirDocs];
+                    const uint32_t b = doc % kDirDocs;
+                    const uint64_t bits = (uint64_t)e.x | ((uint64_t)e.y << 32);
+                    hit = ((bits >> b) & 1ull) != 0ull;
+                    const uint32_t below = (uint32_t)__popcll(bits & ((1ull << b) - 1ull));
+                    hbits = stream[d_first + (hit ? e.z + below : 0u)].y;
+                } else {
+                    const uint32_t cell = doc / kSkipDocs;
+                    uint32_t a = d_skips[cell];
+                    uint32_t n = d_skips[cell + 1u] - a;
+#pragma unroll
+                    for (int step = 0; step < 4; step++) {
+                        const uint32_t s8 = (n + 7u) >> 3;
+                        nat_u2 pv[7];
+#pragma unroll
+                        for (int i = 0; i < 7; i++) {
+                            const uint32_t e = (uint32_t)(i + 1) * s8;
+                            pv[i] = stream[a + ((e <= n && e != 0u) ? e - 1u : 0u)];
+                        }
+                        uint32_t c = 0u;
+#pragma unroll
+                        for (int i = 0; i < 7; i++) {
+                            const uint32_t e = (uint32_t)(i + 1) * s8;
+                            const bool valid = e <= n && e != 0u;
+                            c += (valid && pv[i].x < doc) ? 1u : 0u;
+                            if (valid && pv[i].x == doc) { hit = true; hbits = pv[i].y; }
+                        }
+                        const bool closed = c < 7u && (c + 1u) * s8 <= n;
+                        a += c * s8;
+                        n = (n == 0u) ? 0u : (closed ? s8 - 1u : n - c * s8);
+                    }
                 }
                 hit = hit && own;
                 if (hit) vals[lane] = vals[lane] + d_wq * __uint_as_float(hbits);
diff --git a/nextsearch-api_amd/csrc/ns_internal.h b/nextsearch-api_amd/csrc/ns_internal.h
--- a/nextsearch-api_amd/csrc/ns_internal.h
+++ b/nextsearch-api_amd/csrc/ns_internal.h
@@ -73,6 +73,8 @@
     uint32_t dterm;
 };
 static constexpr uint32_t kRowLen = 64;
+static constexpr uint32_t kDirDocs = 64;
+static constexpr uint32_t kDirTermBits = 4;
 
 struct DevGroup {
     uint64_t bounds_off;
diff --git a/nextsearch-api_amd/csrc/ns_plan.hpp b/nextsearch-api_amd/csrc/ns_plan.hpp
--- a/nextsearch-api_amd/csrc/ns_plan.hpp
+++ b/nextsearch-api_amd/csrc/ns_plan.hpp
@@ -46,6 +46,7 @@
 static constexpr uint64_t kItemTermGeneral = 4000, kItemTermThin = 3000, kItemTermTile = 8000;
 static constexpr uint32_t kRowMinUsers = 4, kRowCellPostings = 65536;
 static constexpr uint32_t kRowMaxTerms = 16;
+static constexpr uint32_t kDirMinCount = 16384, kRowReach = 32;
 
 inline std::string vformat(const char* fmt, va_list ap) {
     char buf[512];
@@ -97,9 +98,11 @@
     struct Imp { uint32_t count, idf_bits; };
     struct Skip { uint32_t count, entry; };
     struct Bmx { uint32_t count, idf_bits, entry; };
+    struct Dir { uint32_t count, entry; };
     ListTable<Imp> imp;
     ListTable<Skip> skip;
     ListTable<Bmx> bmx;
+    ListTable<Dir> dir;
     std::map<uint32_t, uint32_t> share_lists;
     bool share_admit(uint32_t first, uint32_t count) {
         auto it = share_lists.lower_bound(first);
@@ -117,6 +120,10 @@
     }
     uint32_t skip_of(uint32_t first, uint32_t count) const {
         const Skip* e = skip.find(first);
+        return e && e->count == count ? e->entry + 1u : 0u;
+    }
+    uint32_t dir_of(uint32_t first, uint32_t count) const {
+        const Dir* e = dir.find(first);
         return e && e->count == count ? e->entry + 1u : 0u;
     }
     uint32_t bmx_of(uint32_t first, uint32_t count, uint32_t idf_bits) const {
@@ -162,6 +169,7 @@
     int row_mode = 0;
     uint32_t row_min_users = kRowMinUsers;
     uint32_t row_cell_postings = kRowCellPostings;
+    uint32_t row_reach = kRowReach;
 };
 
 inline size_t place_at(size_t& off, size_t bytes) {
@@ -172,7 +180,8 @@
 
 
 struct HostGroup { DevGroup g; uint32_t query; uint64_t cost; uint64_t cmax; uint64_t work; bool wave; uint8_t cls; bool fast_div; bool signed_in; bool grid; bool merge2;
-                   uint32_t rkey1; };
+                   uint32_t rkey1;
+                   uint32_t rdir; };
 
 struct RowKey {
     uint32_t seg, first, count, idf_bits, w_bits;
@@ -186,7 +195,7 @@
     }
 };
 struct RowKeyEnt { RowKey key; uint32_t users, skip, cells, prod_begin, rank; bool on; };
-struct RowCand { uint32_t group, dterm, skip, key; };
+struct RowCand { uint32_t group, dterm, skip, key, dir; };
 
 constexpr uint32_t kOrderBuckets = 2048;
 inline uint32_t order_bucket(uint64_t c) {
@@ -371,13 +380,15 @@
                         hg.merge2 = auto_mode && C.use_merge && hg.cls == 0 && hg.g.term_count == 2 && rest * C.merge_ratio >= hg.cmax;
                         if (hg.merge2) hg.work = hg.cmax + rest * kWorkMerge;
                     }
-                    if (row_try && hg.wave && hg.cls == 1 && !hg.signed_in && hg.g.term_count <= kRowMaxTerms && hg.cmax >= kSkipMinCount &&
+                    const bool reach_ = hg.cls == 0 && !hg.merge2 && C.row_reach < 32 && (hg.cost - hg.cmax) * C.row_reach <= hg.cmax;
+                    if (row_try && hg.wave && (hg.cls == 1 || reach_) && !hg.signed_in && hg.g.term_count <= kRowMaxTerms && hg.cmax >= kSkipMinCount &&
                         sv.n_docs > 0 && !sv.lists->skip.empty() && !(C.use_pruning && hg.g.term_count == 1)) {
                         const DevTerm* dt = S.dterms.data() + hg.g.term_begin;
                         uint32_t d = 0;
                         while (dt[d].count != hg.cmax) d++;
                         const uint32_t sk = sv.lists->skip_of((uint32_t)dt[d].list_off, dt[d].count);
-                        if (sk) S.rcand.push_back(RowCand{(uint32_t)S.groups.size(), d, sk, 0u});
+                        const uint32_t dr = sv.lists->dir_of((uint32_t)dt[d].list_off, dt[d].count);
+                        if (sk && (hg.cls == 1 || dr)) S.rcand.push_back(RowCand{(uint32_t)S.groups.size(), d, sk, 0u, dr});
                     }
                     if (!hg.wave) {
                         hg.g.bounds_off = S.bounds_total;
@@ -525,7 +536,7 @@
             for (unsigned s = 0; s < width; s++) {
                 PrepSlice& S = slices[s];
                 for (const RowCand& c : S.rcand)
-                    if (rkeys[c.key].on) S.groups[c.group].rkey1 = c.key + 1u;
+                    if (rkeys[c.key].on) { S.groups[c.group].rkey1 = c.key + 1u; S.groups[c.group].rdir = c.dir; }
             }
         }
 
@@ -600,7 +611,7 @@
                             if (rk) {
                                 uint32_t d = 0;
                                 while (dt[d].count != hg.cmax) d++;
-                                S.ritems.push_back(DevRItem{it, rk->prod_begin + i, d});
+                                S.ritems.push_back(DevRItem{it, rk->prod_begin + i, d | (hg.rdir << kDirTermBits)});
                                 S.rbucket.push_back((uint16_t)bucket);
                                 S.hist[2 * kOrderBuckets + bucket]++;
                                 continue;
diff --git a/nextsearch-api_amd/csrc/ns_row_kernel.hip b/nextsearch-api_amd/csrc/ns_row_kernel.hip
--- a/nextsearch-api_amd/csrc/ns_row_kernel.hip
+++ b/nextsearch-api_amd/csrc/ns_row_kernel.hip
@@ -27,7 +27,8 @@
     RowArgs ra;
     ra.hits = row_hits + (size_t)ri.row * kRowLen;
     ra.nhits = row_nhits[ri.row];
-    ra.dterm = ri.dterm;
+    ra.dterm = ri.dterm & ((1u << kDirTermBits) - 1u);
+    ra.dir = ri.dterm >> kDirTermBits;
     ra.stats = stats;
     if (dscore_body<HK / 2, 64, false, CB, true, 0, true>(it, terms, segs, s_tbl, s_vals, s_mcnt, s_cand, s_tab, s_aux, out_hits, out_nhits,
                                                           out_found, K, lane, ra))
diff --git a/nextsearch-api_amd/csrc/ns_wave_kernel.hip b/nextsearch-api_amd/csrc/ns_wave_kernel.hip
--- a/nextsearch-api_amd/csrc/ns_wave_kernel.hip
+++ b/nextsearch-api_amd/csrc/ns_wave_kernel.hip
@@ -321,6 +321,8 @@
 typedef const __attribute__((address_space(1))) nat_u2* gp_u2;
 typedef const __attribute__((address_space(1))) float* gp_f32;
 typedef const __attribute__((address_space(1))) uint32_t* gp_u32;
+typedef unsigned int nat_u4 __attribute__((ext_vector_type(4)));
+typedef const __attribute__((address_space(1))) nat_u4* gp_u4;
 
 __device__ __forceinline__ uint2 item_list_range(const DevWItem& it, const DevSeg& seg, const DevTerm& tm) {
     uint32_t cur = 0, end = tm.count;
diff --git a/nextsearch-api_amd/nsbind.py b/nextsearch-api_amd/nsbind.py
--- a/nextsearch-api_amd/nsbind.py
+++ b/nextsearch-api_amd/nsbind.py
@@ -59,7 +59,7 @@
     "ns_ctx_create", "ns_ctx_destroy", "ns_ctx_set_stream", "ns_last_error", "ns_device_name",
     "ns_segment_upload", "ns_segment_release", "ns_segment_upload_begin", "ns_segment_upload_append", "ns_segment_upload_end", "ns_search_batch", "ns_batch_prepare",
     "ns_batch_bind_outputs", "ns_batch_run", "ns_batch_stream", "ns_batch_gap_ms", "ns_batch_sync", "ns_batch_fetch", "ns_batch_get_info",
-    "ns_batch_destroy", "ns_set_tuning", "ns_segment_build_impacts", "ns_ctx_use_impacts", "ns_ctx_set_host_threads", "ns_ctx_set_overlap", "ns_segment_build_packed", "ns_ctx_use_packed", "ns_segment_build_skips", "ns_ctx_use_skips", "ns_segment_build_blockmax", "ns_ctx_use_pruning", "ns_ctx_use_merge", "ns_ctx_share_scores", "ns_ctx_share_rows", "ns_batch_row_stats",
+    "ns_batch_destroy", "ns_set_tuning", "ns_segment_build_impacts", "ns_ctx_use_impacts", "ns_ctx_set_host_threads", "ns_ctx_set_overlap", "ns_segment_build_packed", "ns_ctx_use_packed", "ns_segment_build_skips", "ns_ctx_use_skips", "ns_segment_build_blockmax", "ns_ctx_use_pruning", "ns_ctx_use_merge", "ns_ctx_share_scores", "ns_ctx_share_rows", "ns_batch_row_stats", "ns_segment_dir_bytes",
     "ns_invert_forward", "ns_segment_upload_inverted", "ns_merge_rank_rows", "ns_sem_upload", "ns_sem_release", "ns_sem_topk",
     "ns_ac_upload", "ns_ac_suggest", "ns_ac_release", "ns_ac_build_fuzzy", "ns_ac_fuzzy", "ns_ac_fuzzy_prefix",
     "ns_forward_build", "ns_forward_get_info", "ns_forward_fetch", "ns_forward_destroy",
@@ -194,6 +194,11 @@
         if hasattr(L, "ns_ctx_share_rows"):
             L.ns_ctx_share_rows.argtypes = [vp, i32]
             L.ns_batch_row_stats.argtypes = [vp, vp]
+        if hasattr(L, "ns_segment_dir_bytes"):
+            L.ns_segment_dir_bytes.argtypes = [vp]
+            L.ns_segment_dir_bytes.restype = u64
+            L.ns_debug_read_dir.argtypes = [vp, u64, vp, u32]
+            L.ns_debug_read_dir.restype = C.c_longlong
         L.ns_sem_upload.argtypes = [vp, vp, u32, u32, C.POINTER(vp)]
         L.ns_sem_release.argtypes = [vp, vp]
         L.ns_sem_topk.argtypes = [vp, vp, vp, u32, u32, C.c_float, vp, vp, vp, vp, vp, vp]
```

New measurement: 8.914 million. About the same (-0.7%).
